# W298/Surtr

Measured on AMD Instinct MI355X. Metric: fragments/sec, higher is better.
Workload: dtype f32

## Files before the change

include/surtr_hip.h:

```cpp
#ifndef SURTR_HIP_H
#define SURTR_HIP_H

#include <stddef.h>
#include <stdint.h>

#ifdef __cplusplus
extern "C" {
#endif

typedef struct surtr_ctx surtr_ctx;

enum {
    SURTR_OK = 0,
    SURTR_E_INVALID = 1,
    SURTR_E_TOPOLOGY = 2,
    SURTR_E_CAPACITY = 3,
    SURTR_E_HIP = 4,
    SURTR_E_STATE = 5,
    SURTR_E_NOGPU = 6
};

enum {
    SURTR_EVT_REFIT = 1,
    SURTR_EVT_RENDER = 2
};

typedef struct surtr_counts {
    uint32_t n_frag;
    uint32_t mesh_verts, mesh_nbrs;
    uint32_t conv_verts, conv_nbrs;
    uint32_t n_idx;
    uint32_t n_pairs;
    uint32_t status;
    uint32_t n_failed;
} surtr_counts;

typedef struct surtr_fragments {
    int32_t* frag_ids;
    uint32_t* mesh_vert_off;
    float* mesh_pos;
    uint32_t* mesh_nbr_off;
    int32_t* mesh_nbr;
    uint32_t* conv_vert_off;
    float* conv_pos;
    uint32_t* conv_nbr_off;
    int32_t* conv_nbr;
    float* vnc;
    uint32_t* idx_off;
    uint32_t* idx;
    uint32_t* frag_status;
} surtr_fragments;

int surtr_create(int device, surtr_ctx** out);
void surtr_destroy(surtr_ctx* ctx);
const char* surtr_strerror(int code);
const char* surtr_last_error(surtr_ctx* ctx);
int surtr_set_stream(surtr_ctx* ctx, void* hip_stream);
int surtr_get_stream(surtr_ctx* ctx, void** hip_stream);
int surtr_set_events_in_flight(surtr_ctx* ctx, uint32_t n);
int surtr_set_scratch(surtr_ctx* ctx, uint32_t max_verts, uint32_t max_nbrs);
int surtr_set_arena(surtr_ctx* ctx, uint64_t verts, uint64_t nbrs, uint64_t idx);

int surtr_set_profiling(surtr_ctx* ctx, int on);
int surtr_kernel_times(surtr_ctx* ctx, float ms[16]);
int surtr_kernel_history(surtr_ctx* ctx, float ms[16], int slot[16], uint32_t* n);
int surtr_queue_stats(surtr_ctx* ctx, uint32_t out[128]);
int surtr_pair_status(surtr_ctx* ctx, uint32_t n_pairs, uint32_t* status);
int surtr_event_pair_costs(surtr_ctx* ctx, uint32_t n_pairs, uint32_t* cost);

int surtr_upload_pieces(surtr_ctx* ctx, uint32_t n_pieces,
                        const uint32_t* mesh_vert_off, const float* mesh_pos,
                        const uint32_t* mesh_nbr_off, const int32_t* mesh_nbr,
                        const uint32_t* conv_vert_off, const float* conv_pos,
                        const uint32_t* conv_nbr_off, const int32_t* conv_nbr);

int surtr_upload_pattern(surtr_ctx* ctx, uint32_t n_cells, const uint32_t* face_off, const float* v012);

int surtr_build_cells(surtr_ctx* ctx, uint32_t n_groups, const uint32_t* group_seed_off, const double* seeds,
                      uint32_t* n_faces, uint32_t* n_face_verts);
int surtr_download_cells(surtr_ctx* ctx, uint32_t* cell_face_off, int32_t* face_gen, uint32_t* face_vert_off, double* verts, float* v012);

int surtr_place_cells(surtr_ctx* ctx, const float scale[3], const float translate[3]);
int surtr_place_cells_impacts(surtr_ctx* ctx, uint32_t n_impacts, const float* scale3, const float* translate3);
int surtr_download_planes(surtr_ctx* ctx, int impacts, uint32_t cap, uint32_t* n, float* planes);

#define SURTR_CELLS_ALL 0xFFFFFFFFu
int surtr_pattern_store(surtr_ctx* ctx, uint32_t* id);
int surtr_pattern_count(surtr_ctx* ctx, uint32_t* n);
int surtr_pattern_info(surtr_ctx* ctx, uint32_t id, uint32_t* n_cells, uint32_t* n_faces);
int surtr_pattern_clear(surtr_ctx* ctx);
int surtr_pattern_select(surtr_ctx* ctx, uint32_t id);
int surtr_place_cells_patterns(surtr_ctx* ctx, uint32_t n_impacts, const uint32_t* pattern_id, const float* scale3, const float* translate3);
int surtr_placed_cells(surtr_ctx* ctx, uint32_t cap, uint32_t* n, uint32_t* cell_base);

int surtr_upload_planes(surtr_ctx* ctx, uint32_t n_cells, const uint32_t* plane_off, const float* planes);

int surtr_fracture_event(surtr_ctx* ctx, uint32_t cell_begin, uint32_t cell_end,
                         const uint8_t* outside, uint32_t flags, surtr_counts* counts);

int surtr_fracture_event_async(surtr_ctx* ctx, uint32_t cell_begin, uint32_t cell_end,
                               const uint8_t* outside, uint32_t flags);
int surtr_event_counts(surtr_ctx* ctx, surtr_counts* counts);

int surtr_fracture_pairs_async(surtr_ctx* ctx, uint32_t n_pairs, const uint32_t* pair_cell, const uint32_t* pair_piece,
                               uint32_t flags);
int surtr_place_cells_groups(surtr_ctx* ctx, uint32_t n_groups, const uint32_t* group_cell_off, const float* scale3,
                             const float* translate3);

int surtr_place_cells_in_pieces(surtr_ctx* ctx, uint32_t n_groups, const uint32_t* group_cell_off);

size_t surtr_event_blob_bytes(const surtr_counts* counts);
int surtr_event_pack_dev(surtr_ctx* ctx, void* dev_blob, size_t capacity_bytes);
int surtr_blob_unpack_host(const void* host_blob, size_t bytes, surtr_counts* counts, surtr_fragments* out);
int surtr_event_download(surtr_ctx* ctx, surtr_fragments* out);

int surtr_clip_polyhedron(surtr_ctx* ctx, uint32_t nv, const float* pos, const uint32_t* nbr_off, const int32_t* nbr,
                          uint32_t n_planes, const float* planes,
                          uint32_t* out_nv, uint32_t* out_nh, float* out_pos, uint32_t* out_nbr_off, int32_t* out_nbr);

int surtr_refit_solid(surtr_ctx* ctx, uint32_t mesh_nv, const float* mesh_pos, const uint32_t* mesh_nbr_off, const int32_t* mesh_nbr,
                      uint32_t conv_nv, const float* conv_pos, const uint32_t* conv_nbr_off, const int32_t* conv_nbr,
                      uint32_t* out_nv, uint32_t* out_nh, float* out_pos, uint32_t* out_nbr_off, int32_t* out_nbr);
int surtr_extract_faces(surtr_ctx* ctx, uint32_t nv, const float* pos, const uint32_t* nbr_off, const int32_t* nbr,
                        uint32_t* n_faces, uint32_t* n_face_idx, uint32_t* face_off, int32_t* face_idx);
int surtr_triangulate(surtr_ctx* ctx, uint32_t nv, const float* pos, const uint32_t* nbr_off, const int32_t* nbr, int is_convex,
                      const float color[3], float* vnc, uint32_t* n_idx, uint32_t* idx);

int surtr_load_fragments(surtr_ctx* ctx, uint32_t n,
                         const uint32_t* mesh_vert_off, const float* mesh_pos, const uint32_t* mesh_nbr_off, const int32_t* mesh_nbr,
                         const uint32_t* conv_vert_off, const float* conv_pos, const uint32_t* conv_nbr_off, const int32_t* conv_nbr,
                         const int32_t* frag_ids);
int surtr_event_triangulate(surtr_ctx* ctx, int is_convex);

int surtr_transform_pieces(surtr_ctx* ctx, uint32_t n_pieces, const float* world);
int surtr_pieces_from_event(surtr_ctx* ctx, const uint8_t* keep, uint32_t* n_pieces);
int surtr_download_piece(surtr_ctx* ctx, uint32_t piece, int set, uint32_t* out_nv, uint32_t* out_nh, float* out_pos,
                         uint32_t* out_nbr_off, int32_t* out_nbr);
enum {
    SURTR_DERIVED_LLEN = 0,
    SURTR_DERIVED_TRI = 1,
    SURTR_DERIVED_RAD = 2,
    SURTR_DERIVED_BOX = 3,
    SURTR_DERIVED_PERM = 4,
    SURTR_DERIVED_POSR_S = 5,
    SURTR_DERIVED_BSPH = 6,
    SURTR_DERIVED_BSPH2 = 7,
    SURTR_DERIVED_BSPH3 = 8,
    SURTR_DERIVED_IPERM = 9,
    SURTR_DERIVED_ROW_S = 10,
    SURTR_DERIVED_DUP = 11,
    SURTR_DERIVED_BO = 12,
    SURTR_DERIVED_BO2 = 13,
    SURTR_DERIVED_BO3 = 14,
    SURTR_DERIVED_BUILD = 15,
    SURTR_DERIVED_COUNT = 16
};
int surtr_pieces_derived(surtr_ctx* ctx, int set, int which, void* out, size_t capacity_bytes, size_t* bytes);
int surtr_upload_stats(surtr_ctx* ctx, float* ms, uint32_t* n_alloc);
int surtr_handover_stats(surtr_ctx* ctx, uint32_t out[8]);
int surtr_regroup_stats(surtr_ctx* ctx, uint32_t out[8]);
int surtr_pair_order(surtr_ctx* ctx, uint32_t cap, uint32_t* n, uint32_t* order);

int surtr_neighbors_from_mesh(uint32_t nv, uint32_t n_tris, const int32_t* tris, uint32_t* nbr_off, int32_t* nbr);

int surtr_neighbors_from_mesh_dev(surtr_ctx* ctx, uint32_t nv, uint32_t n_tris, const int32_t* tris, uint32_t* nbr_off, int32_t* nbr,
                                  float* kernel_ms);

int surtr_voronoi_cells(uint32_t n, const double* seeds, uint32_t* n_faces, uint32_t* n_face_verts,
                        uint32_t* cell_face_off, int32_t* face_gen, uint32_t* face_vert_off, double* verts);

int surtr_hull_normals(uint32_t n, const float* points, uint32_t limit, uint32_t capacity, float* normals, uint32_t* count);

int surtr_kdop_ach_planes(uint32_t n, const float* points, uint32_t k, const float* normals, double max_axis_scale,
                          float plane_gap_inv, float* planes);

int surtr_plane_from_points(const float p0[3], const float p1[3], const float p2[3], float plane[4]);

int surtr_kdop_planes(uint32_t n, const float* points, uint32_t k, const float* normals, float* planes);

int surtr_moments(uint32_t nv, const float* pos, const uint32_t* nbr_off, const int32_t* nbr, double* volume, float centroid[3]);

int surtr_read_obj(const char* path, const float scale[3], const float translate[3], uint32_t cap_verts, uint32_t cap_tris,
                   float* pos, int32_t* tris, uint32_t* n_verts, uint32_t* n_tris);
int surtr_write_obj(const char* path, uint32_t n_frag, const int32_t* frag_ids, const uint32_t* mesh_vert_off, const float* vnc,
                    const uint32_t* idx_off, const uint32_t* idx);

int surtr_convex_out_of_sphere(uint32_t nv, const float* pos, const uint32_t* nbr_off, const int32_t* nbr, uint32_t n_sphere,
                               const float* sphere_points, const float origin[3], float radius, int* out);

int surtr_regroup(uint32_t n_pieces, uint32_t n_outside, const int32_t* piece_cell,
                  const uint32_t* conv_vert_off, const float* conv_pos, const uint32_t* conv_nbr_off, const int32_t* conv_nbr,
                  int partial, uint32_t n_sphere, const float* sphere_points, const float origin[3], float radius,
                  uint32_t* n_compounds, uint32_t* compound_off, int32_t* compound_piece);

int surtr_event_regroup(surtr_ctx* ctx, int partial, uint32_t n_sphere, const float* sphere_points, const float origin[3], float radius,
                        uint32_t* n_pieces, uint32_t* n_compounds, uint32_t* compound_off, int32_t* compound_piece);
int surtr_event_regroup_bodies(surtr_ctx* ctx, int partial, uint32_t n_sphere, const float* sphere_points, const float origin[3], float radius,
                               uint32_t* n_pieces, uint32_t* n_compounds, uint32_t* compound_off, int32_t* compound_piece,
                               uint32_t* n_bodies, uint32_t* body_compound_off);
int surtr_event_regroup_impacts(surtr_ctx* ctx, int partial, uint32_t n_impacts, const uint32_t* sphere_off, const float* sphere_points,
                                const float* origins, const float* radii, uint32_t* n_pieces, uint32_t* n_compounds, uint32_t* compound_off,
                                int32_t* compound_piece, uint32_t* n_bodies, uint32_t* body_compound_off);

int surtr_event_regroup_impacts_partial(surtr_ctx* ctx, const uint8_t* partial, uint32_t n_impacts, const uint32_t* sphere_off, const float* sphere_points,
                                        const float* origins, const float* radii, uint32_t* n_pieces, uint32_t* n_compounds, uint32_t* compound_off,
                                        int32_t* compound_piece, uint32_t* n_bodies, uint32_t* body_compound_off);

int surtr_event_refit(surtr_ctx* ctx);

int surtr_set_refit_point_limit(surtr_ctx* ctx, uint32_t n);
int surtr_get_refit_point_limit(surtr_ctx* ctx, uint32_t* n);
int surtr_hull_normals_device(surtr_ctx* ctx, uint32_t n, const float* points, uint32_t limit, uint32_t capacity, float* normals, uint32_t* count);
int surtr_coord_key(float x, uint32_t* neg, uint64_t* scaled);

typedef struct surtr_mass {
    double volume;
    double mass;
    double com[3];
    double inertia[6];
    uint32_t nv;
    uint32_t status;
} surtr_mass;

int surtr_event_mass_dev(surtr_ctx* ctx, int set, float density, void* dev_out, size_t capacity_bytes);
int surtr_pieces_mass_dev(surtr_ctx* ctx, int set, float density, void* dev_out, size_t capacity_bytes);
int surtr_event_mass(surtr_ctx* ctx, int set, float density, uint32_t* n, surtr_mass* out);
int surtr_pieces_mass(surtr_ctx* ctx, int set, float density, uint32_t* n, surtr_mass* out);
int surtr_combine_mass(uint32_t n_compounds, const uint32_t* compound_off, const int32_t* compound_piece, const surtr_mass* pieces,
                       surtr_mass* out);

typedef struct surtr_ray_hit {
    int32_t piece;
    uint32_t status;
    float t;
    float pos[3];
    float normal[3];
    uint32_t reserved[3];
} surtr_ray_hit;
enum {
    SURTR_RAY_STARTS_INSIDE = 1,
// ... 153 lines not shown
```

surtr_amd/csrc/pieces_dev.hip:

```cpp
#include <chrono>
#include <cstring>

#include "surtr_ctx.h"
#include <hipcub/hipcub.hpp>

namespace {

__device__ __forceinline__ int32_t ring_prev(const int32_t* r, uint32_t len, int32_t who)
{
    uint32_t k = 0;
    while (k < len && r[k] != who) ++k;
    return k == 0 ? r[len - 1] : r[k - 1];
}

__device__ __forceinline__ uint32_t piece_of(const uint32_t* __restrict__ vo, uint32_t n, uint32_t v)
{
    uint32_t lo = 0, hi = n;
    while (hi - lo > 1u) { const uint32_t mid = (lo + hi) >> 1; if (vo[mid] <= v) lo = mid; else hi = mid; }
    return lo;
}

__global__ void k_piece_check(uint32_t V, uint32_t n, const uint32_t* __restrict__ vo, const uint32_t* __restrict__ loff,
                              const int32_t* __restrict__ nbr, uint32_t* __restrict__ llen, uint32_t check, uint32_t* __restrict__ err,
                              uint8_t* __restrict__ dup, uint32_t H)
{
    const uint32_t v = blockIdx.x * blockDim.x + threadIdx.x;
    if (v >= V) return;
    const uint32_t lo = loff[v], hi = loff[v + 1];
    if (hi < lo || hi > H) { atomicMax(err, (uint32_t)SURTR_E_INVALID); llen[v] = 0; return; }
    const uint32_t deg = hi - lo;
    llen[v] = deg;
    const uint32_t p = piece_of(vo, n, v), a = vo[p], m = vo[p + 1] - a;
    for (uint32_t j = lo + 1u; j < hi; ++j)
        for (uint32_t q = lo; q < j; ++q) if (nbr[q] == nbr[j]) { dup[p] = 1; j = hi; break; }
    if (!check) return;
    if (deg < 3u) { atomicMax(err, (uint32_t)SURTR_E_TOPOLOGY); return; }
    const int32_t lv = (int32_t)(v - a);
    for (uint32_t j = lo; j < hi; ++j)
    {
        const int32_t u = nbr[j];
        if (u < 0 || (uint32_t)u >= m || u == lv) { atomicMax(err, (uint32_t)SURTR_E_TOPOLOGY); return; }
        const uint32_t ulo = loff[a + (uint32_t)u], uhi = loff[a + (uint32_t)u + 1];
        if (uhi > H) { atomicMax(err, (uint32_t)SURTR_E_INVALID); return; }
        bool back = false;
        for (uint32_t q = ulo; q < uhi && q >= ulo; ++q) if (nbr[q] == lv) { back = true; break; }
        if (!back) { atomicMax(err, (uint32_t)SURTR_E_TOPOLOGY); return; }
    }
}

__global__ void k_piece_tri_rad(uint32_t V, uint32_t n, const uint32_t* __restrict__ vo, const float* __restrict__ pos,
                                const uint32_t* __restrict__ loff, const int32_t* __restrict__ nbr, uint8_t* __restrict__ tri,
                                float* __restrict__ rad, const uint32_t* __restrict__ gate)
{
    const uint32_t v = blockIdx.x * blockDim.x + threadIdx.x;
    if (v >= V) return;
    if (gate && *gate) return;
    const uint32_t p = piece_of(vo, n, v), a = vo[p], m = vo[p + 1] - a;
    const int32_t lv = (int32_t)(v - a);
    auto ring = [&](int32_t x) { return nbr + loff[a + (uint32_t)x]; };
    auto rlen = [&](int32_t x) { return loff[a + (uint32_t)x + 1] - loff[a + (uint32_t)x]; };
    const uint32_t lo = loff[v], hi = loff[v + 1];
    bool t = true;
    for (uint32_t j = lo; j < hi; ++j)
    {
        const int32_t x = nbr[j];
        const int32_t y = ring_prev(ring(x), rlen(x), lv);
        if (y == lv || ring_prev(ring(y), rlen(y), x) != lv) { t = false; break; }
    }
    tri[v] = t ? 1 : 0;
    const double px = pos[3 * (size_t)v], py = pos[3 * (size_t)v + 1], pz = pos[3 * (size_t)v + 2];
    auto dist = [&](int32_t x) {
        const size_t g = a + (uint32_t)x;
        const double dx = px - (double)pos[3 * g], dy = py - (double)pos[3 * g + 1], dz = pz - (double)pos[3 * g + 2];
        return sqrt(dx * dx + dy * dy + dz * dz);
    };
    double r = 0.0;
    for (uint32_t j = lo; j < hi; ++j)
    {
        const double d = dist(nbr[j]);
        r = d > r ? d : r;
        if (!t)
        {
            int32_t prev = lv, cur = nbr[j]; uint32_t steps = 0;
            while (cur != lv && steps++ < m)
            {
                const double d2 = dist(cur);
                r = d2 > r ? d2 : r;
                const int32_t nx = ring_prev(ring(cur), rlen(cur), prev);
                prev = cur; cur = nx;
            }
        }
    }
    rad[v] = (float)(r * 1.000001) + 1e-30f;
}

__global__ __launch_bounds__(SURTR_WG) void k_piece_box(uint32_t n, const uint32_t* __restrict__ vo, const float* __restrict__ pos, float* __restrict__ box)
{
    __shared__ float part[SURTR_NWAVE][6];
    const uint32_t p = blockIdx.x;
    if (p >= n) return;
    const uint32_t a = vo[p], b = vo[p + 1];
    float lo[3] = {3.0e38f, 3.0e38f, 3.0e38f}, hi[3] = {-3.0e38f, -3.0e38f, -3.0e38f};
    for (uint32_t v = a + threadIdx.x; v < b; v += group_size())
        for (int c = 0; c < 3; ++c) { const float x = pos[3 * (size_t)v + c]; lo[c] = x < lo[c] ? x : lo[c]; hi[c] = x > hi[c] ? x : hi[c]; }
    for (int d = SURTR_LANES / 2; d >= 1; d >>= 1)
        for (int c = 0; c < 3; ++c)
        {
            const float ol = __shfl_down(lo[c], d, SURTR_LANES), oh = __shfl_down(hi[c], d, SURTR_LANES);
            lo[c] = ol < lo[c] ? ol : lo[c]; hi[c] = oh > hi[c] ? oh : hi[c];
        }
    if (lane_id() == 0) for (int c = 0; c < 3; ++c) { part[wave_id()][c] = lo[c]; part[wave_id()][3 + c] = hi[c]; }
    __syncthreads();
    if (threadIdx.x == 0)
    {
        for (uint32_t w = 1; w < group_waves(); ++w)
            for (int c = 0; c < 3; ++c)
            {
                lo[c] = part[w][c] < lo[c] ? part[w][c] : lo[c];
                hi[c] = part[w][3 + c] > hi[c] ? part[w][3 + c] : hi[c];
            }
        for (int c = 0; c < 3; ++c) { box[6 * p + c] = lo[c]; box[6 * p + 3 + c] = hi[c]; }
    }
}

__global__ void k_piece_keys(uint32_t V, uint32_t n, const uint32_t* __restrict__ vo, const float* __restrict__ pos,
                             const float* __restrict__ box, unsigned long long* __restrict__ key, uint32_t* __restrict__ val)
{
    const uint32_t v = blockIdx.x * blockDim.x + threadIdx.x;
    if (v >= V) return;
    const uint32_t p = piece_of(vo, n, v);
// ... 76 lines not shown
        const double dx = s.x - (double)cx, dy = s.y - (double)cy, dz = s.z - (double)cz;
        const double d = sqrt(dx * dx + dy * dy + dz * dz) + (double)s.w;
        R = d > R ? d : R;
    }
    upper[g] = make_float4(cx, cy, cz, (float)(R * 1.000001) + 1e-30f);
}

__global__ void k_piece_iperm(uint32_t V, uint32_t n, const uint32_t* __restrict__ vo, const uint32_t* __restrict__ perm, uint32_t* __restrict__ iperm)
{
    const uint32_t i = blockIdx.x * blockDim.x + threadIdx.x;
    if (i >= V) return;
    const uint32_t p = piece_of(vo, n, i), a = vo[p];
    iperm[a + perm[i]] = i - a;
}
__global__ void k_piece_row_s(uint32_t V, uint32_t n, const uint32_t* __restrict__ vo, const uint32_t* __restrict__ perm,
                              const uint32_t* __restrict__ loff, const uint32_t* __restrict__ llen, const int32_t* __restrict__ nbr,
                              const uint8_t* __restrict__ tri, const uint32_t* __restrict__ iperm, SRow* __restrict__ row_s)
{
    const uint32_t i = blockIdx.x * blockDim.x + threadIdx.x;
    if (i >= V) return;
    const uint32_t p = piece_of(vo, n, i), a = vo[p], m = vo[p + 1] - a;
    const uint32_t g = a + perm[i];
    const uint32_t lo = loff[g], len = llen[g];
    uint32_t h[8];
    h[0] = (len <= 7u ? len : 0x40u) | (tri[g] ? 0u : 0x80u);
    for (uint32_t j = 0; j < 7u; ++j)
    {
        uint32_t e = 0xFFFFu;
        if (len <= 7u && j < len)
        {
            const int32_t u = nbr[lo + j];
            if (u >= 0 && (uint32_t)u < m) { const uint32_t x = iperm[a + (uint32_t)u]; e = x < 0xFFFFu ? x : 0xFFFFu; }
        }
        h[1u + j] = e;
    }
    SRow r;
    for (int q = 0; q < 4; ++q) r.w[q] = h[2 * q] | (h[2 * q + 1] << 16);
    row_s[i] = r;
}

__global__ void k_transform(uint32_t V, uint32_t n, const uint32_t* __restrict__ vo, const float* __restrict__ world, float* __restrict__ pos,
                            uint32_t v0, uint32_t p0)
{
    const uint32_t v = v0 + blockIdx.x * blockDim.x + threadIdx.x;
    if (v >= V) return;
    const float* W = world + 16 * (size_t)(piece_of(vo, n, v) - p0);
    float r[3];
    transform_coord(W, pos[3 * (size_t)v], pos[3 * (size_t)v + 1], pos[3 * (size_t)v + 2], r);
    pos[3 * (size_t)v] = r[0]; pos[3 * (size_t)v + 1] = r[1]; pos[3 * (size_t)v + 2] = r[2];
}

struct FromEvent { const uint32_t* frag; const uint32_t* vo[2]; const uint32_t* ho[2]; };
__global__ __launch_bounds__(SURTR_WG) void k_pieces_from_frags(uint32_t n, FromEvent E, const FragRec* __restrict__ frags, Arena A,
                                                                float* mpos, uint32_t* mloff, int32_t* mnbr, float* cpos, uint32_t* cloff, int32_t* cnbr)
{
    const uint32_t p = blockIdx.x >> 1, set = blockIdx.x & 1u;
    if (p >= n) return;
    const FragRec fr = frags[E.frag[p]];
    const uint32_t sv = set ? fr.cv_off : fr.mv_off, nv = set ? fr.cv_n : fr.mv_n, sh = set ? fr.ch_off : fr.mh_off, nh = set ? fr.ch_n : fr.mh_n;
    const uint32_t dv = E.vo[set][p], dh = E.ho[set][p];
    float* pos = set ? cpos : mpos; uint32_t* loff = set ? cloff : mloff; int32_t* nbr = set ? cnbr : mnbr;
    for (uint32_t i = threadIdx.x; i < 3u * nv; i += group_size()) pos[3 * (size_t)dv + i] = A.pos[3 * (size_t)sv + i];
    for (uint32_t v = threadIdx.x; v < nv; v += group_size()) loff[dv + v] = dh + (A.loff[sv + v] - sh);
    for (uint32_t e = threadIdx.x; e < nh; e += group_size()) nbr[dh + e] = A.nbr[sh + e];
    if (p + 1u == n && threadIdx.x == 0) loff[dv + nv] = dh + nh;
}

static inline uint32_t up_count(uint32_t m) { return (m + SURTR_SPH_FAN - 1u) / SURTR_SPH_FAN; }

}

namespace pieces {

int reserve_set(surtr_ctx* ctx, PieceSet& S, uint32_t n, uint32_t V, uint32_t H, uint32_t NB)
{
    if (grow_pieces(ctx, S.pos, 3 * (size_t)V + 3) || grow_pieces(ctx, S.loff, (size_t)V + 1) || grow_pieces(ctx, S.llen, V) ||
        grow_pieces(ctx, S.nbr, (size_t)H + 1) || grow_pieces(ctx, S.vo, n + 1) || grow_pieces(ctx, S.tri, V) || grow_pieces(ctx, S.rad, V) ||
        grow_pieces(ctx, S.perm, V) || grow_pieces(ctx, S.posr_s, (size_t)V + 1) || grow_pieces(ctx, S.bsph, NB + 1) ||
        grow_pieces(ctx, S.bo, n + 1) || grow_pieces(ctx, S.box, 6 * (size_t)n) || grow_pieces(ctx, S.key, V) || grow_pieces(ctx, S.key2, V) ||
        grow_pieces(ctx, S.val, V) || grow_pieces(ctx, S.dup, n + 1) || grow_pieces(ctx, S.iperm, V) || grow_pieces(ctx, S.row_s, (size_t)V + 1) ||
        grow_pieces(ctx, S.bsph2, (size_t)NB / SURTR_SPH_FAN + n + 1) || grow_pieces(ctx, S.bo2, n + 1) ||
        grow_pieces(ctx, S.bsph3, (size_t)NB / (SURTR_SPH_FAN * SURTR_SPH_FAN) + n + 1) || grow_pieces(ctx, S.bo3, n + 1))
        return SURTR_E_HIP;
    return SURTR_OK;
}

int derive_set(surtr_ctx* ctx, PieceSet& S, uint32_t n, uint32_t V, const std::vector<uint32_t>& bo_h, bool check, uint32_t H)
{
    hipStream_t st = ctx->stream;
    const uint32_t NB = bo_h[n];
    HIPCHK(hipMemcpyAsync(S.bo, bo_h.data(), (size_t)(n + 1) * 4, hipMemcpyHostToDevice, st));
    const dim3 blk(256), gridV((V + 255) / 256);
    HIPCHK(hipMemsetAsync(S.dup, 0, (size_t)n + 1, st));
    hipLaunchKernelGGL(k_piece_check, gridV, blk, 0, st, V, n, S.vo, S.loff, S.nbr, S.llen, check ? 1u : 0u, ctx->d_upload_err, S.dup, check ? H : 0xFFFFFFFFu);
    hipLaunchKernelGGL(k_piece_tri_rad, gridV, blk, 0, st, V, n, S.vo, S.pos, S.loff, S.nbr, S.tri, S.rad,
                       check ? (const uint32_t*)ctx->d_upload_err.p : (const uint32_t*)nullptr);
    hipLaunchKernelGGL(k_piece_box, dim3(n), dim3(SURTR_WG), 0, st, n, S.vo, S.pos, S.box);
    hipLaunchKernelGGL(k_piece_keys, gridV, blk, 0, st, V, n, S.vo, S.pos, S.box, S.key, S.val);
    int end_bit = 32;
    while (end_bit < 64 && (n >> (end_bit - 32)) != 0u) ++end_bit;
    size_t tmp_bytes = 0;
    if (hipcub::DeviceRadixSort::SortPairs(nullptr, tmp_bytes, S.key.p, S.key2.p, S.val.p, S.perm.p, (int)V, 0, end_bit, st) != hipSuccess) return SURTR_E_HIP;
    int rc = grow_pieces(ctx, ctx->sort_tmp, tmp_bytes + 16);
    if (rc) return rc;
    if (hipcub::DeviceRadixSort::SortPairs(ctx->sort_tmp.p, tmp_bytes, S.key.p, S.key2.p, S.val.p, S.perm.p, (int)V, 0, end_bit, st) != hipSuccess) return SURTR_E_HIP;
    hipLaunchKernelGGL(k_piece_sorted, gridV, blk, 0, st, V, n, S.vo, S.pos, S.rad, S.perm, S.posr_s);
    if (NB) hipLaunchKernelGGL(k_piece_spheres, dim3((NB + 255) / 256), blk, 0, st, NB, n, S.vo, S.bo, S.posr_s, S.bsph);
    std::vector<uint32_t> bo2(n + 1, 0u), bo3(n + 1, 0u);
    for (uint32_t p = 0; p < n; ++p) { bo2[p + 1] = bo2[p] + up_count(bo_h[p + 1] - bo_h[p]); bo3[p + 1] = bo3[p] + up_count(bo2[p + 1] - bo2[p]); }
    HIPCHK(hipMemcpyAsync(S.bo2, bo2.data(), (size_t)(n + 1) * 4, hipMemcpyHostToDevice, st));
    HIPCHK(hipMemcpyAsync(S.bo3, bo3.data(), (size_t)(n + 1) * 4, hipMemcpyHostToDevice, st));
    if (bo2[n]) hipLaunchKernelGGL(k_piece_spheres_up, dim3((bo2[n] + 255) / 256), blk, 0, st, bo2[n], n, S.bo, S.bo2, S.bsph, S.bsph2);
    if (bo3[n]) hipLaunchKernelGGL(k_piece_spheres_up, dim3((bo3[n] + 255) / 256), blk, 0, st, bo3[n], n, S.bo2, S.bo3, S.bsph2, S.bsph3);
    hipLaunchKernelGGL(k_piece_iperm, gridV, blk, 0, st, V, n, S.vo, S.perm, S.iperm);
    hipLaunchKernelGGL(k_piece_row_s, gridV, blk, 0, st, V, n, S.vo, S.perm, S.loff, S.llen, S.nbr, S.tri, S.iperm, S.row_s);
    HIPCHK(hipGetLastError());
    return SURTR_OK;
}

int host_offsets(uint32_t n, const uint32_t* vo, const uint32_t* off, std::vector<uint32_t>& ho)
{
    if (vo[0] != 0) return SURTR_E_INVALID;
    for (uint32_t p = 0; p < n; ++p)
    {
        const uint32_t a = vo[p], b = vo[p + 1];
        if (b < a || b - a < 4 || b - a >= (1u << 24)) return SURTR_E_INVALID;
        if (off[b] < off[a]) return SURTR_E_INVALID;
    }
    ho.resize(n + 1);
    for (uint32_t p = 0; p <= n; ++p) ho[p] = off[vo[p]];
    return SURTR_OK;
}

int vet_solids(surtr_ctx* ctx, uint32_t n, uint32_t V, uint32_t H, const uint32_t* vo, const uint32_t* loff, const int32_t* nbr, uint32_t* llen, uint8_t* dup)
{
    hipStream_t st = ctx->stream;
    HIPCHK(hipMemsetAsync(dup, 0, (size_t)n + 1, st));
    hipLaunchKernelGGL(k_piece_check, dim3((V + 255) / 256), dim3(256), 0, st, V, n, vo, loff, nbr, llen, 1u, ctx->d_upload_err.p, dup, H);
    HIPCHK(hipGetLastError());
    return SURTR_OK;
}

std::vector<uint32_t> sphere_offsets(uint32_t n, const uint32_t* vo)
{
    std::vector<uint32_t> bo(n + 1, 0u);
    for (uint32_t p = 0; p < n; ++p) bo[p + 1] = bo[p] + (vo[p + 1] - vo[p] + SURTR_SB - 1u) / SURTR_SB;
    return bo;
}

void set_piece_stats(surtr_ctx* ctx, uint32_t n, const uint32_t* mvo, const uint32_t* mho, const uint32_t* cvo, const uint32_t* cho)
{
    uint32_t vmax = 0, hmax = 0, cvmax = 0, chmax = 0, small = 0, vmin = 0xFFFFFFFFu;
    for (uint32_t i = 0; i < n; ++i)
    {
        vmax = std::max(vmax, mvo[i + 1] - mvo[i]); vmin = std::min(vmin, mvo[i + 1] - mvo[i]); hmax = std::max(hmax, mho[i + 1] - mho[i]);
        cvmax = std::max(cvmax, cvo[i + 1] - cvo[i]); chmax = std::max(chmax, cho[i + 1] - cho[i]);
        if (surtr_fits_half((mvo[i + 1] - mvo[i]) / 4u, (mho[i + 1] - mho[i]) / 4u)) ++small;
    }
    ctx->vmin = n ? vmin : 0u;
    ctx->n_pieces = n; ctx->vmax = std::max(vmax, cvmax); ctx->hmax = std::max(hmax, chmax); ctx->cvmax = cvmax; ctx->chmax = chmax;
    ctx->tot_mv = mvo[n]; ctx->tot_mh = mho[n]; ctx->pair_order_count = 0;
    ctx->half_on = 4ull * small >= 3ull * n;
    if (const char* e = getenv("SURTR_HALF")) ctx->half_on = atoi(e) != 0;
    ctx->have_event = false; ctx->frags_of_pieces = false;
    ctx->scene_off.assign({0u, n}); ctx->scene_event_compound.clear();
    scene_reset_poses(ctx);
    ctx->h_vo[0].assign(mvo, mvo + n + 1); ctx->h_ho[0].assign(mho, mho + n + 1);
    ctx->h_vo[1].assign(cvo, cvo + n + 1); ctx->h_ho[1].assign(cho, cho + n + 1);
}

int finish_upload(surtr_ctx* ctx, uint32_t n, bool check)
{
    const int rc = grow_pieces(ctx, ctx->d_outside, n);
    if (rc) return rc;
    uint32_t err = 0;
    HIPCHK(hipMemcpyAsync(&err, ctx->d_upload_err, 4, hipMemcpyDeviceToHost, ctx->stream));
    HIPCHK(hipStreamSynchronize(ctx->stream));
    if (check && err) { ctx->n_pieces = 0; return (int)err; }
    return SURTR_OK;
// ... 144 lines not shown
    if (g >= n) return;
    for (int c = 0; c < 3; ++c)
    {
        const float lo = box[6 * g + c], hi = box[6 * g + 3 + c];
        scale3[3 * g + c] = hi - lo;
        shift3[3 * g + c] = (float)(((double)hi + (double)lo) / 2.0);
    }
}

int surtr_place_cells_in_pieces(surtr_ctx* ctx, uint32_t n_groups, const uint32_t* group_cell_off)
{
    if (!ctx || !n_groups || !group_cell_off) return SURTR_E_INVALID;
    if (!ctx->n_pieces || !ctx->d_v012) return SURTR_E_STATE;
    if (n_groups != ctx->n_pieces) return SURTR_E_INVALID;
    (void)hipSetDevice(ctx->device);
    int rc = grow_pieces(ctx, ctx->d_group_xf, (size_t)6 * n_groups);
    if (rc) return rc;
    float* sc = ctx->d_group_xf; float* sh = sc + 3 * (size_t)n_groups;
    hipLaunchKernelGGL(k_group_boxes, dim3((n_groups + 255) / 256), dim3(256), 0, ctx->stream, n_groups, ctx->mset.box, sc, sh);
    HIPCHK(hipGetLastError());
    return surtr_place_cells_groups_dev(ctx, n_groups, group_cell_off, sc, sh);
}

int surtr_download_piece(surtr_ctx* ctx, uint32_t piece, int set, uint32_t* out_nv, uint32_t* out_nh, float* out_pos, uint32_t* out_off, int32_t* out_nbr)
{
    if (!ctx || set < 0 || set > 1) return SURTR_E_INVALID;
    if (!ctx->n_pieces) return SURTR_E_STATE;
    if (piece >= ctx->n_pieces) return SURTR_E_INVALID;
    (void)hipSetDevice(ctx->device);
    const PieceSet& S = set ? ctx->cset : ctx->mset;
    HIPCHK(hipStreamSynchronize(ctx->stream));
    uint32_t vo[2], ho[2];
    HIPCHK(hipMemcpy(vo, S.vo + piece, 8, hipMemcpyDeviceToHost));
    HIPCHK(hipMemcpy(&ho[0], S.loff + vo[0], 4, hipMemcpyDeviceToHost));
    HIPCHK(hipMemcpy(&ho[1], S.loff + vo[1], 4, hipMemcpyDeviceToHost));
    const uint32_t nv = vo[1] - vo[0], nh = ho[1] - ho[0];
    if (out_nv) *out_nv = nv;
    if (out_nh) *out_nh = nh;
    if (out_pos) HIPCHK(hipMemcpy(out_pos, S.pos + 3 * (size_t)vo[0], (size_t)nv * 12, hipMemcpyDeviceToHost));
    if (out_off)
    {
        HIPCHK(hipMemcpy(out_off, S.loff + vo[0], ((size_t)nv + 1) * 4, hipMemcpyDeviceToHost));
        for (uint32_t v = 0; v <= nv; ++v) out_off[v] -= ho[0];
    }
    if (out_nbr && nh) HIPCHK(hipMemcpy(out_nbr, S.nbr + ho[0], (size_t)nh * 4, hipMemcpyDeviceToHost));
    return SURTR_OK;
}

int surtr_upload_stats(surtr_ctx* ctx, float* ms, uint32_t* n_alloc)
{
    if (!ctx) return SURTR_E_INVALID;
    if (ms) *ms = ctx->upload_ms;
    if (n_alloc) *n_alloc = ctx->upload_allocs;
    return SURTR_OK;
}

int surtr_handover_stats(surtr_ctx* ctx, uint32_t out[8])
{
    if (!ctx || !out) return SURTR_E_INVALID;
    (void)hipSetDevice(ctx->device);
    HIPCHK(hipStreamSynchronize(ctx->stream));
    if (ctx->stream2) HIPCHK(hipStreamSynchronize(ctx->stream2));
    if (ctx->stream3) HIPCHK(hipStreamSynchronize(ctx->stream3));
    uint32_t c[CUR_HO_WORDS] = {};
    if (ctx->arena.cursors) HIPCHK(hipMemcpy(c, ctx->arena.cursors + CUR_HO_PUSHED, sizeof(c), hipMemcpyDeviceToHost));
    for (uint32_t k = 0; k < CUR_HO_WORDS; ++k) out[k] = c[k];
    out[6] = ctx->max_wg;
    out[7] = (uint32_t)ctx->d_hlist.cap;
    return SURTR_OK;
}

int surtr_pair_order(surtr_ctx* ctx, uint32_t cap, uint32_t* n, uint32_t* order)
{
    if (!ctx || !n) return SURTR_E_INVALID;
    (void)hipSetDevice(ctx->device);
    *n = ctx->d_pair_order ? ctx->pair_order_count : 0u;
    if (!order || *n == 0u) return SURTR_OK;
    if (cap < *n) return SURTR_E_CAPACITY;
    HIPCHK(hipStreamSynchronize(ctx->stream));
    HIPCHK(hipMemcpy(order, ctx->d_pair_order, (size_t)*n * 4, hipMemcpyDeviceToHost));
    return SURTR_OK;
}

int surtr_pieces_derived(surtr_ctx* ctx, int set, int which, void* out, size_t capacity_bytes, size_t* bytes)
{
    if (!ctx || set < 0 || set > 1 || !bytes || which < 0 || which >= SURTR_DERIVED_COUNT) return SURTR_E_INVALID;
    const uint32_t build[2] = {SURTR_SB, SURTR_SPH_FAN};
    const void* src = nullptr; size_t b = 0;
    if (which == SURTR_DERIVED_BUILD) b = sizeof(build);
    else
    {
        if (!ctx->n_pieces) return SURTR_E_STATE;
        const PieceSet& S = set ? ctx->cset : ctx->mset;
        const uint32_t n = ctx->n_pieces; const size_t V = ctx->h_vo[set][n];
        const std::vector<uint32_t> bo = sphere_offsets(n, ctx->h_vo[set].data());
        size_t nb2 = 0, nb3 = 0;
        for (uint32_t p = 0; p < n; ++p) { const uint32_t a = up_count(bo[p + 1] - bo[p]); nb2 += a; nb3 += up_count(a); }
        switch (which)
        {
        case SURTR_DERIVED_LLEN:   src = S.llen.p;   b = V * 4; break;
        case SURTR_DERIVED_TRI:    src = S.tri.p;    b = V; break;
        case SURTR_DERIVED_RAD:    src = S.rad.p;    b = V * 4; break;
        case SURTR_DERIVED_BOX:    src = S.box.p;    b = (size_t)n * 24; break;
        case SURTR_DERIVED_PERM:   src = S.perm.p;   b = V * 4; break;
        case SURTR_DERIVED_POSR_S: src = S.posr_s.p; b = V * 16; break;
        case SURTR_DERIVED_BSPH:   src = S.bsph.p;   b = (size_t)bo[n] * 16; break;
        case SURTR_DERIVED_BSPH2:  src = S.bsph2.p;  b = nb2 * 16; break;
        case SURTR_DERIVED_BSPH3:  src = S.bsph3.p;  b = nb3 * 16; break;
        case SURTR_DERIVED_IPERM:  src = S.iperm.p;  b = V * 4; break;
        case SURTR_DERIVED_ROW_S:  src = S.row_s.p;  b = V * 16; break;
        case SURTR_DERIVED_DUP:    src = S.dup.p;    b = n; break;
        case SURTR_DERIVED_BO:     src = S.bo.p;     b = ((size_t)n + 1) * 4; break;
        case SURTR_DERIVED_BO2:    src = S.bo2.p;    b = ((size_t)n + 1) * 4; break;
        default:                   src = S.bo3.p;    b = ((size_t)n + 1) * 4; break;
        }
    }
    *bytes = b;
    if (!out) return SURTR_OK;
    if (capacity_bytes < b) return SURTR_E_CAPACITY;
    if (!src) { memcpy(out, build, b); return SURTR_OK; }
    (void)hipSetDevice(ctx->device);
    HIPCHK(hipStreamSynchronize(ctx->stream));
    if (b) HIPCHK(hipMemcpy(out, src, b, hipMemcpyDeviceToHost));
    return SURTR_OK;
}

}
```

surtr_amd/csrc/small_clip.h:

```cpp
#pragma once
#include "clip_core.h"

#define SC_V 192u
#define SC_H 640u
#define SC_FALLBACK 101

namespace surtr {

template <uint32_t CAPV, uint32_t CAPH, class WORD = uint32_t>
struct ScSolidT
{
    typedef WORD Word;
    static constexpr uint32_t kVwSh = sizeof(WORD) == 4 ? 16u : 12u, kReSh = sizeof(WORD) == 4 ? 16u : 8u;
    static_assert(CAPV <= (1u << kReSh) && CAPH <= (1u << kVwSh), "a vertex id / a ring offset fits its field");
    float pos[3 * CAPV];
    WORD vw[CAPV];
    WORD re[CAPH];
};
typedef ScSolidT<SC_V, SC_H> ScSolid;

template <uint32_t CAPV, uint32_t CAPH, class WORD = uint32_t>
struct ScLdsT
{
    static_assert(CAPV % 4u == 0 && CAPV <= 0x7FFFu && CAPH <= 0xFFFFu, "16-bit indices, 4-byte arrays");
    static constexpr uint32_t kV = CAPV, kH = CAPH;
    typedef ScSolidT<CAPV, CAPH, WORD> Solid;
    Solid buf[2];
    int8_t c[CAPV];
    uint16_t km[CAPV];
    uint16_t mp[CAPV];
    uint16_t noff[CAPV];
    uint16_t succ[CAPV], pred[CAPV];
    uint32_t nv[2], flag;
#ifdef SURTR_STAMP
    unsigned long long tph[8];
#endif
};
typedef ScLdsT<SC_V, SC_H> ScLds;

template <class SH, class LDS>
__device__ inline int small_clip(const SolidIn in, const uint32_t F, const SH& sh, LDS& L, uint32_t* which, uint32_t* stop = nullptr)
{
    typedef typename LDS::Solid ScSolid;
    constexpr uint32_t CAPV = LDS::kV, CAPH = LDS::kH;
    constexpr uint32_t VS = ScSolid::kVwSh, VM = (1u << VS) - 1u, RS = ScSolid::kReSh, RM = (1u << RS) - 1u;
    const uint32_t lane = lane_id();
    const uint32_t V = in.nv;
#ifdef SURTR_STAMP
    unsigned long long sc_t0 = __builtin_readcyclecounter();
    if (lane == 0) for (int q = 0; q < 8; ++q) L.tph[q] = 0;
#define SC_STAMP(i) do { if (lane == 0) { const unsigned long long t1 = __builtin_readcyclecounter(); L.tph[i] += t1 - sc_t0; sc_t0 = t1; } } while (0)
#else
#define SC_STAMP(i) do { } while (0)
#endif
    if (stop != nullptr) *stop = 0xFFFFFFFFu;
    if (V == 0 || V > CAPV) return SC_FALLBACK;
    const uint32_t hbase = in.loff[0], H = in.loff[V - 1u] + in.llen[V - 1u] - hbase;
    if (H > CAPH) return SC_FALLBACK;
    bool odd = false;
    for (uint32_t v = lane; v < V; v += SURTR_LANES)
    {
        ScSolid& S = L.buf[0];
        S.pos[3 * v] = in.pos[3 * v]; S.pos[3 * v + 1] = in.pos[3 * v + 1]; S.pos[3 * v + 2] = in.pos[3 * v + 2];
        const uint32_t lo = in.loff[v] - hbase, deg = in.llen[v];
        if (deg > 15u || deg < 3u) odd = true;
        const uint32_t dl = deg > 15u ? 15u : deg;
        S.vw[v] = lo | (dl << VS);
        const int32_t* r = in.nbr + in.loff[v];
        for (uint32_t j = 0; j < dl && lo + j < CAPH; ++j)
        {
            if ((uint32_t)r[j] >= V) odd = true;
            S.re[lo + j] = (uint32_t)r[j] & RM;
            for (uint32_t jj = 0; jj < j; ++jj) if (r[jj] == r[j]) odd = true;
        }
    }
    if (__ballot(odd) != 0ull) return SC_FALLBACK;
    __syncthreads();
    for (uint32_t v = lane; v < V; v += SURTR_LANES)
    {
        ScSolid& S = L.buf[0];
        const uint32_t w = S.vw[v], lo = w & VM, deg = w >> VS;
        for (uint32_t j = 0; j < deg; ++j)
        {
            const uint32_t e = S.re[lo + j] & RM;
            const uint32_t we = S.vw[e], elo = we & VM, edeg = we >> VS;
            uint32_t q = 0;
            while (q < edeg && (S.re[elo + q] & RM) != v) ++q;
            if (q >= edeg) odd = true;
            S.re[lo + j] = e | (q << RS);
        }
    }
    if (__ballot(odd) != 0ull) return SC_FALLBACK;
    __syncthreads();
    SC_STAMP(0);
#define SC_GIVE_UP do { if (stop != nullptr) { *stop = k; *which = cur; if (lane == 0) L.nv[cur] = nv; __syncthreads(); } return SC_FALLBACK; } while (0)
    uint32_t cur = 0, nv = V;
    for (uint32_t k = 0; k < F && nv != 0u; ++k)
    {
        const float4 pl = sh.planes[k];
        ScSolid& S = L.buf[cur]; ScSolid& N = L.buf[cur ^ 1u];
        bool zero = false, cut = false, keep = false;
        for (uint32_t v = lane; v < nv; v += SURTR_LANES)
        {
            const int c = side_of(plane_dist(pl, S.pos[3 * v], S.pos[3 * v + 1], S.pos[3 * v + 2]));
            L.c[v] = (int8_t)c;
            zero = zero || c == 0; cut = cut || c < 0; keep = keep || c > 0;
        }
        const bool anyCut = __ballot(cut) != 0ull;
        if (__ballot(keep) == 0ull) { if (!anyCut) SC_GIVE_UP; nv = 0; break; }
        if (!anyCut) continue;
        if (__ballot(zero) != 0ull) SC_GIVE_UP;
        __syncthreads();
        SC_STAMP(1);
        uint32_t carryM = 0, carryK = 0, carryH = 0;
        for (uint32_t v0 = 0; v0 < nv; v0 += SURTR_LANES)
        {
            const uint32_t v = v0 + lane;
            uint32_t mask = 0, isKept = 0, deg = 0;
            if (v < nv)
            {
                const uint32_t w = S.vw[v], lo = w & VM;
                deg = w >> VS;
                if (L.c[v] > 0) isKept = 1u;
                else
                    for (uint32_t j = 0; j < deg; ++j) if (L.c[S.re[lo + j] & RM] > 0) mask |= 1u << j;
            }
            const uint32_t cnt = (uint32_t)__builtin_popcount(mask);
            const uint2 inc = wave_incl_scan2(make_uint2(cnt | (isKept << 16), isKept ? deg : 0u));
            if (v < nv)
            {
                L.km[v] = (uint16_t)mask;
                L.mp[v] = isKept ? (uint16_t)(carryK + (inc.x >> 16) - 1u) : (uint16_t)(0x8000u | (carryM + (inc.x & 0xFFFFu) - cnt));
                L.noff[v] = (uint16_t)(carryH + inc.y - (isKept ? deg : 0u));
            }
            const uint32_t tx = lane_bcast(inc.x, SURTR_LANES - 1u), ty = lane_bcast(inc.y, SURTR_LANES - 1u);
            carryM += tx & 0xFFFFu; carryK += tx >> 16; carryH += ty;
        }
        const uint32_t M = carryM, nKeep = carryK, HK = carryH;
        if (nKeep + M > CAPV || HK + 3u * M > CAPH) SC_GIVE_UP;
        if (nKeep + M < 4u) { nv = 0; break; }
        for (uint32_t t = lane; t < M; t += SURTR_LANES) L.pred[t] = 0xFFFFu;
        __syncthreads();
        SC_STAMP(2);
        bool bad = false;
        for (uint32_t v = lane; v < nv; v += SURTR_LANES)
        {
            uint32_t mask = L.c[v] < 0 ? L.km[v] : 0u;
            if (!mask) continue;
            uint32_t t = L.mp[v] & 0x7FFFu;
            const uint32_t wv = S.vw[v];
            for (; mask; mask &= mask - 1u, ++t)
            {
                uint32_t cv = v, w = wv, slot = (uint32_t)__builtin_ctz(mask), steps = 0, end = 0xFFFFu;
                while (steps++ <= nv)
                {
                    const uint32_t len = w >> VS;
                    const uint32_t p = slot == 0u ? len - 1u : slot - 1u;
                    const uint32_t rw = S.re[(w & VM) + p];
                    const uint32_t e = rw & RM;
                    if (L.c[e] > 0) { end = (L.mp[cv] & 0x7FFFu) + (uint32_t)__builtin_popcount(L.km[cv] & ((1u << p) - 1u)); break; }
                    cv = e; slot = rw >> RS; w = S.vw[e];
                }
                if (end == 0xFFFFu || end == t) { bad = true; continue; }
                L.succ[t] = (uint16_t)end;
                L.pred[end] = (uint16_t)t;
            }
        }
        if (__ballot(bad) != 0ull) SC_GIVE_UP;
        __syncthreads();
        SC_STAMP(3);
        for (uint32_t t = lane; t < M; t += SURTR_LANES) if (L.pred[t] == 0xFFFFu || L.pred[L.succ[t]] != t || L.pred[t] == L.succ[t]) bad = true;
        if (__ballot(bad) != 0ull) SC_GIVE_UP;
        SC_STAMP(4);
        for (uint32_t v = lane; v < nv; v += SURTR_LANES)
        {
            const uint32_t w = S.vw[v], lo0 = w & VM, deg = w >> VS;
            if (L.c[v] > 0)
// ... 95 lines not shown
```

surtr_amd/csrc/surtr_ctx.h:

```cpp
#pragma once
#include <algorithm>
#include <chrono>
#include <cstdint>
#include <cstdlib>
#include <string>
#include <vector>

#include "../../include/surtr_hip.h"
#include "clip_core.h"

using namespace surtr;

struct PairRec
{
    uint32_t cv_off, cv_n, ch_off, ch_n;
    uint32_t mv_off, mv_n, mh_off, mh_n;
    uint32_t ni, isl_off;
    uint32_t status;
    uint32_t img_fmt, img_off, img_n, img_h, img_pc;
    uint32_t cv_bad;
};

enum { IMG_NONE = 0,
       IMG_NARROW = 1,
// ... 30 lines not shown
    uint32_t mv_off, mv_n, mh_off, mh_n;
    uint32_t cv_off, cv_n, ch_off, ch_n;
    uint32_t idx_off, idx_n;
    uint32_t o_mv, o_mh, o_cv, o_ch, o_idx;
};

struct Arena
{
    float* pos; uint32_t* loff; uint32_t* llen; int32_t* nbr; uint32_t* idx;
    uint2* isl;
    uint32_t capV, capH, capI, capIsl;
    uint32_t* cursors;
};

enum : uint32_t
{
    CUR_V = 0,
    CUR_H = 1,
    CUR_I = 2,
    CUR_ISL = 3,
    CUR_Q_CLIP = 4,
    CUR_STATUS = 5,
    CUR_Q_REFIT = 6,
    CUR_Q_FACES = 7,
    CUR_Q_CONVEX = 8,
    CUR_Q_PREP = 9,
    CUR_IMG = 10,
    CUR_Q_BIG = 11,
    CUR_Q_HALF = 12,
    CUR_Q_RETRY = 13,
    CUR_FLAGGED_FRAGS = 14,
    CUR_FLAGGED_PAIRS = 15,
    CUR_CLS_CLIP = 16,
    CUR_CLS_FRAG = 32,
    CUR_CLS_PREP = 48,
    CUR_CLS_HALF = 64,
    CUR_RETRY_N = CUR_CLS_HALF,
    CUR_CVX_RESUMED = 78,
    CUR_REFIT_RESUMED = 79,
    CUR_CVX_TOOK = 80,
    CUR_REFIT_TOOK = 82,
    CUR_BIG_QUOTA = 84,
    CUR_FACES2_N = 85,
    CUR_Q_FACES2 = 86,
    CUR_CVX_GAVE_UP = 87,
    CUR_REC_TOOK = 88,
    CUR_REC_HANDED = 89,
    CUR_LIT_TOO_LARGE = 90,
    CUR_REC_IMAGES = 91,
    CUR_SORTED_SEL = 92,
    CUR_REC_SPENT = 93,
    CUR_CATCH_CLIPPED = 94,
    CUR_UNREFITTED = 95,
    CUR_WC_WHY = 96,
    CUR_Q_CONVEX2 = 125,
    CUR_STATS_WORDS = 128,
    CUR_HO_PUSHED = 146,
    CUR_HO_STARTED = 147,
    CUR_HO_SIGNED_OFF = 148,
    CUR_HO_POLL_SLOT = 149,
    CUR_Q_CATCH = 150,
    CUR_Q_SWEEP = 151,
    CUR_HO_WORDS = 6,
    CUR_COUNT = 256
};
static_assert(CUR_V == 0 && CUR_H == 1 && CUR_I == 2 && CUR_ISL == 3 && CUR_STATUS == 5 && CUR_CLS_CLIP == 16 && CUR_CLS_FRAG == 32 &&
              CUR_CLS_PREP == 48 && CUR_CLS_HALF == 64 && CUR_REC_TOOK == 88 && CUR_REC_HANDED == 89 && CUR_LIT_TOO_LARGE == 90 &&
              CUR_UNREFITTED == 95 && CUR_WC_WHY == 96, "include/surtr_hip.h publishes these slots of surtr_queue_stats by number");
static_assert(CUR_STATS_WORDS <= CUR_COUNT && CUR_Q_SWEEP + 1 == CUR_HO_PUSHED + CUR_HO_WORDS && CUR_HO_PUSHED + CUR_HO_WORDS <= CUR_COUNT &&
              CUR_Q_FACES2 == CUR_FACES2_N + 1, "slot map");

struct alignas(16) SRow { uint32_t w[4]; };

struct Pieces
{
    const float* mpos; const uint32_t* mloff; const uint32_t* mllen; const int32_t* mnbr; const uint32_t* mvo; const uint8_t* mtri; const float* mrad;
    const uint32_t* mperm; const float4* mposr_s; const float4* mbsph; const uint32_t* mbo;
    const float* cpos; const uint32_t* cloff; const uint32_t* cllen; const int32_t* cnbr; const uint32_t* cvo; const uint8_t* ctri; const float* crad;
    const uint32_t* cperm; const float4* cposr_s; const float4* cbsph; const uint32_t* cbo;
    uint32_t n;
    const uint8_t* mdup; const uint8_t* cdup;
    const SRow* mrow_s; const uint32_t* miperm;
    const float4* mbsph2; const uint32_t* mbo2; const float4* mbsph3; const uint32_t* mbo3;
};

struct ScratchPool
{
    char* base; size_t per_wg;
    uint32_t CV, CH, VMAX;
};

struct Scratch
{
    float* pos;
    uint32_t* g_loff; uint32_t* g_llen; int8_t* g_comp; uint32_t* g_ring;
    uint32_t* g_succ; uint32_t* g_pred; uint32_t* g_pcnt;
    uint32_t* aux0; uint32_t* aux1; uint32_t* aux2; uint32_t* aux3;
    int8_t* g_gcomp;
    uint2* blk;
    unsigned long long* gmask; uint2* gblk;
    float* t_pos; uint32_t* t_loff; uint32_t* t_llen; int8_t* t_comp; uint32_t* t_ring;
    uint32_t CV, CH;
};

__device__ static Scratch carve(const ScratchPool& P, uint32_t wg)
{
    Scratch S;
    char* p = P.base + (size_t)wg * P.per_wg;
    auto take = [&](size_t bytes) { char* r = p; p += (bytes + 255) & ~(size_t)255; return r; };
    S.pos = (float*)take((size_t)P.CV * 12);
    S.g_loff = (uint32_t*)take((size_t)P.CV * 4);
    S.g_llen = (uint32_t*)take((size_t)P.CV * 4);
    S.g_comp = (int8_t*)take((size_t)P.CV);
    S.g_ring = (uint32_t*)take((size_t)P.CH * 4);
    S.g_succ = (uint32_t*)take((size_t)P.CV * 4);
    S.g_pred = (uint32_t*)take((size_t)P.CV * 4);
    S.g_pcnt = (uint32_t*)take((size_t)P.CV * 4);
    const size_t AV = P.CV > P.VMAX ? P.CV : P.VMAX;
    S.aux0 = (uint32_t*)take(AV * 4);
    S.aux1 = (uint32_t*)take((size_t)P.CV * 4);
    S.aux2 = (uint32_t*)take(AV * 4);
    S.aux3 = (uint32_t*)take((size_t)P.CV * 4);
    S.g_gcomp = (int8_t*)take((size_t)P.CV);
    S.blk = (uint2*)take((size_t)(P.CV / SURTR_LANES + 4) * 8);
    S.gmask = (unsigned long long*)take((size_t)(P.VMAX / SURTR_LANES + 2) * 8);
    S.gblk = (uint2*)take((size_t)(P.VMAX / SURTR_LANES + 2) * 8);
    S.t_pos = (float*)take((size_t)P.CV * 12); S.t_loff = (uint32_t*)take((size_t)P.CV * 4); S.t_llen = (uint32_t*)take((size_t)P.CV * 4);
    S.t_comp = (int8_t*)take((size_t)P.CV); S.t_ring = (uint32_t*)take((size_t)P.CH * 4);
    S.CV = P.CV; S.CH = P.CH;
    return S;
}

static size_t scratch_bytes_per_wg(uint32_t CV, uint32_t CH, uint32_t VMAX)
{
    auto r = [](size_t b) { return (b + 255) & ~(size_t)255; };
    return 2 * r((size_t)CV * 12) + 9 * r((size_t)CV * 4) + 2 * r((size_t)std::max(CV, VMAX) * 4) + 3 * r((size_t)CV) + 2 * r((size_t)CH * 4) + r((size_t)(CV / SURTR_LANES + 4) * 8) +
           2 * r((size_t)(VMAX / SURTR_LANES + 2) * 8);
}

struct FaceScratch
{
    int32_t* base; size_t per_wg; uint32_t HF;
};

struct surtr_ctx;

template <class T>
struct DevBuf
{
    T* p = nullptr;
    size_t cap = 0;
    DevBuf() = default;
    DevBuf(DevBuf&& o) noexcept : p(o.p), cap(o.cap) { o.p = nullptr; o.cap = 0; }
    DevBuf& operator=(DevBuf&& o) noexcept { if (this != &o) { reset(); p = o.p; cap = o.cap; o.p = nullptr; o.cap = 0; } return *this; }
    ~DevBuf() { reset(); }
    void reset() { if (p) (void)hipFree(p); p = nullptr; cap = 0; }
    operator T*() const { return p; }
    int grow(surtr_ctx* ctx, size_t need, size_t alloc = 0);
};

struct PieceSet
{
    DevBuf<float> pos; DevBuf<uint32_t> loff, llen; DevBuf<int32_t> nbr; DevBuf<uint32_t> vo; DevBuf<uint8_t> tri; DevBuf<float> rad;
    DevBuf<uint32_t> perm; DevBuf<float4> posr_s, bsph; DevBuf<uint32_t> bo;
    DevBuf<float> box; DevBuf<unsigned long long> key, key2; DevBuf<uint32_t> val;
    DevBuf<uint8_t> dup;
    DevBuf<uint32_t> iperm; DevBuf<SRow> row_s;
    DevBuf<float4> bsph2; DevBuf<uint32_t> bo2; DevBuf<float4> bsph3; DevBuf<uint32_t> bo3;
};

struct CellBuffers
{
    DevBuf<double> seeds; DevBuf<uint32_t> goff; DevBuf<char> slots; DevBuf<uint32_t> cfo, cvo;
    DevBuf<int32_t> gen; DevBuf<uint32_t> fvo; DevBuf<double> verts; DevBuf<uint32_t> heads;
    uint32_t n = 0, nf = 0, nfv = 0;
};

#define SURTR_LVS (SURTR_LV / 2u)
#define SURTR_LHS ((SURTR_LH * 11u / 24u) & ~7u)
#ifndef SURTR_HALF_ROOM
#define SURTR_HALF_ROOM 2u
#endif
__host__ __device__ static inline bool fits_half(uint32_t n, uint32_t h, uint32_t capVs) { return SURTR_HALF_ROOM * n <= capVs && SURTR_HALF_ROOM * h <= SURTR_LHS; }
static inline bool surtr_fits_half(uint32_t n, uint32_t h) { return fits_half(n, h, SURTR_LVS); }

struct surtr_ctx
{
    int device = 0;
    bool frags_of_pieces = false;
    uint32_t hw_wg = 512, hw_wg_faces = 1024, hw_wg_prep = 1792, hw_wg_big = 48, budget_vmax = 0xFFFFFFFFu, budget_hmax = 0xFFFFFFFFu;
    uint32_t max_wg = 512, max_wg_faces = 1024, max_wg_small = 2048, max_wg_lean = 3072, max_wg_prep = 1792, max_wg_half = 1024;
    DevBuf<uint32_t> d_hlist;
    uint32_t vmin = 0;
    ScratchPool pool_half{}; uint32_t n_wg_half = 0; DevBuf<char> pool_half_buf;
    bool half_on = false;
    PrepPool prep{nullptr, 0, 0}; uint32_t n_wg_prep = 0; DevBuf<char> prep_buf;
    ImgArena img{nullptr, 0}; DevBuf<char> img_buf;
    DevBuf<uint32_t> d_order;
    DevBuf<uint32_t> d_forder;
    bool wave_big = false;
    uint32_t n_wg_big = 48;
    hipStream_t stream2 = nullptr;
    hipStream_t stream3 = nullptr;
    hipEvent_t ev_prep = nullptr, ev_big = nullptr, ev_half = nullptr, ev_cvx = nullptr;
    uint32_t events_in_flight = 1;
    hipStream_t stream = nullptr;
    std::string err;
    uint32_t n_pieces = 0, vmax = 0, hmax = 0, cvmax = 0, chmax = 0;
    CellBuffers cells;
    PieceSet mset, cset;
    DevBuf<uint32_t> d_upload_err;
    DevBuf<float> d_group_xf;
    DevBuf<float> d_world;
    DevBuf<char> sort_tmp;
    DevBuf<uint32_t> d_from;
    DevBuf<uint32_t> d_qstatus; uint32_t qstatus_n = 0;
    float upload_ms = 0.f; uint32_t upload_allocs = 0;
    std::vector<uint32_t> scene_off;
    std::vector<uint32_t> h_vo[2], h_ho[2];
    std::vector<uint32_t> scene_event_compound;
    std::vector<uint32_t> scene_event_impacts;
    DevBuf<uint32_t> d_outside_list;
    std::vector<uint32_t> h_outside_stage;
    std::vector<float> scene_pose;
    bool scene_dev_stale = true;
    std::vector<double> h_pose_stage; std::vector<uint32_t> h_comp_stage;
    DevBuf<double> d_pose;
    DevBuf<uint32_t> d_piece_comp;
    struct { DevBuf<float> pos; DevBuf<uint32_t> loff; DevBuf<int32_t> nbr; DevBuf<uint32_t> vo; } spare[2];
    DevBuf<int32_t> d_commit_src; DevBuf<uint32_t> d_commit_tab;
    DevBuf<float> d_posef; bool scene_posef_stale = true; std::vector<float> h_posef_stage;
    DevBuf<surtr_bounds> d_bounds_piece;
    DevBuf<char> d_cull;
    struct { DevBuf<float> pos; DevBuf<uint32_t> loff, llen, vo; DevBuf<int32_t> nbr; DevBuf<uint8_t> dup; } stage[2];
    std::vector<uint32_t> h_frag_stage; DevBuf<uint32_t> d_frag_tab;
    float commit_ms[2] = {0.f, 0.f};
    uint32_t regroup_rounds = 0;
    uint64_t tot_mv = 0, tot_mh = 0;
    uint32_t n_cells = 0, n_faces = 0;
    DevBuf<uint32_t> d_cvx_giveup;
    DevBuf<uint32_t> d_pair_order; uint32_t pair_order_begin = 0, pair_order_count = 0;
    bool pair_order_is_list = false;
    DevBuf<float> d_v012; DevBuf<float4> d_planes; DevBuf<uint32_t> d_plane_off;
    std::vector<uint32_t> h_plane_off;
    bool planes_ready = false;
    uint32_t n_impacts_placed = 0;
    DevBuf<float4> d_planes_imp; DevBuf<uint32_t> d_plane_off_imp; DevBuf<float> d_imp_xf;
    std::vector<uint32_t> h_plane_off_imp; std::vector<float> h_imp_xf;
    bool imp_library = false; std::vector<uint32_t> imp_cell_base; uint32_t imp_faces = 0;
    DevBuf<uint32_t> d_imp_tab; std::vector<uint32_t> h_imp_tab;
    struct LibPattern { uint32_t n_cells, n_faces, face_base, off_base; };
// ... 218 lines not shown
```

surtr_amd/csrc/surtr_hip.hip:

```cpp
#include <algorithm>
#include <cmath>
#include <cstdio>
#include <cstdlib>
#include <cstring>
#include <string>
#include <type_traits>
#include <vector>

#include "surtr_ctx.h"
#include "small_clip.h"
#ifndef SC_RESUME
#define SC_RESUME 1
#endif
#include "literal_clip.h"
#include "wave_clip.h"
#include "prep_sorted.h"

template <uint32_t LV, uint32_t LH>
struct alignas(16) LdsTopoT
{
    static_assert(LV % 16 == 0 && LH % 8 == 0, "clip_image copies 16-byte words into these arrays");
    static constexpr uint32_t kLV = LV, kLH = LH;
    alignas(16) uint16_t loff[LV];
    alignas(16) uint8_t llen[LV];
// ... 197 lines not shown
    const uint32_t f = blockIdx.x * blockDim.x + threadIdx.x;
    if (f >= nfaces) return;
    const uint32_t g = face_group[f];
    const float sx = scale3[3 * g], sy = scale3[3 * g + 1], sz = scale3[3 * g + 2];
    const float tx = shift3[3 * g], ty = shift3[3 * g + 1], tz = shift3[3 * g + 2];
    planes[f] = placed_plane(v012 + 9 * f, sx, sy, sz, tx, ty, tz);
}

__global__ void k_place_cells_impacts(uint32_t nfaces, uint32_t n_imp, const float* __restrict__ v012, const float* __restrict__ scale3,
                                      const float* __restrict__ shift3, float4* __restrict__ planes)
{
    const uint32_t f = blockIdx.x * blockDim.x + threadIdx.x;
    if (f >= nfaces) return;
    float v[9];
    for (int i = 0; i < 9; ++i) v[i] = v012[9 * (size_t)f + i];
    for (uint32_t g = 0; g < n_imp; ++g)
    {
        const float sx = scale3[3 * g], sy = scale3[3 * g + 1], sz = scale3[3 * g + 2];
        const float tx = shift3[3 * g], ty = shift3[3 * g + 1], tz = shift3[3 * g + 2];
        planes[(size_t)g * nfaces + f] = placed_plane(v, sx, sy, sz, tx, ty, tz);
    }
}

__global__ void k_place_cells_patterns(uint32_t ntotal, uint32_t n_imp, const uint32_t* __restrict__ face_prefix, const uint32_t* __restrict__ lib_face_base,
                                       const float* __restrict__ lib_v012, const float* __restrict__ scale3, const float* __restrict__ shift3,
                                       float4* __restrict__ planes)
{
    const uint32_t g = blockIdx.x * blockDim.x + threadIdx.x;
    if (g >= ntotal) return;
    uint32_t lo = 0, hi = n_imp;
    while (hi - lo > 1u)
    {
        const uint32_t mid = lo + (hi - lo) / 2u;
        if (face_prefix[mid] <= g) lo = mid; else hi = mid;
    }
    const uint32_t f = g - face_prefix[lo];
    const float* src = lib_v012 + 9 * ((size_t)lib_face_base[lo] + f);
    float v[9];
    for (int i = 0; i < 9; ++i) v[i] = src[i];
    const float sx = scale3[3 * lo], sy = scale3[3 * lo + 1], sz = scale3[3 * lo + 2];
    const float tx = shift3[3 * lo], ty = shift3[3 * lo + 1], tz = shift3[3 * lo + 2];
    planes[g] = placed_plane(v, sx, sy, sz, tx, ty, tz);
}

__device__ __forceinline__ void pair_failed(const Arena& A, int err)
{
    if (err == SURTR_E_TOPOLOGY) atomicAdd(&A.cursors[CUR_FLAGGED_PAIRS], 1u); else atomicMax(&A.cursors[CUR_STATUS], (uint32_t)err);
}

__device__ __forceinline__ uint32_t pair_of_ticket(const Arena& A, const uint32_t* __restrict__ table, uint32_t n_pairs, uint32_t& t, uint32_t class_base,
                                                   int cls_hi, int cls_lo)
{
    uint32_t p = 0xFFFFFFFFu;
    for (int cls = cls_hi; cls >= cls_lo; --cls)
    {
        const uint32_t cnt = A.cursors[class_base + cls];
        if (t < cnt) { p = table[(size_t)cls * n_pairs + t]; break; }
        t -= cnt;
    }
    return p;
}
__device__ __forceinline__ uint32_t take_pair(const Arena& A, const uint32_t* __restrict__ table, uint32_t n_pairs, uint32_t ticket_slot, uint32_t class_base,
                                              int cls_hi, int cls_lo)
{
    uint32_t t = atomicAdd(&A.cursors[ticket_slot], 1u);
    return pair_of_ticket(A, table, n_pairs, t, class_base, cls_hi, cls_lo);
}
struct PairAt { uint32_t cell, piece; };
__device__ __forceinline__ PairAt pair_where(uint32_t p, const uint2* __restrict__ pair_list, uint32_t cell_begin, uint32_t n_pieces)
{
    return PairAt{pair_list ? pair_list[p].x : cell_begin + p / n_pieces, pair_list ? pair_list[p].y : p % n_pieces};
}
__device__ __forceinline__ SolidIn mesh_solid_in(const Pieces& P, uint32_t piece)
{
    const uint32_t m0 = P.mvo[piece];
    return SolidIn{P.mpos + 3 * (size_t)m0, P.mloff + m0, P.mllen + m0, P.mnbr, P.mvo[piece + 1] - m0, P.mtri + m0, P.mrad + m0,
                   P.mperm + m0, P.mposr_s + m0, P.mbsph + P.mbo[piece]};
}
__device__ __forceinline__ SolidIn convex_solid_in(const Pieces& P, uint32_t piece)
{
    const uint32_t c0 = P.cvo[piece];
    return SolidIn{P.cpos + 3 * (size_t)c0, P.cloff + c0, P.cllen + c0, P.cnbr, P.cvo[piece + 1] - c0, P.ctri + c0, P.crad + c0,
                   P.cperm + c0, P.cposr_s + c0, P.cbsph + P.cbo[piece]};
}
__device__ __forceinline__ int finish_pair(const Arena& A, PairRec* __restrict__ pairs, uint32_t p, PairRec& rec, int err)
{
    if (err == 0 && rec.cv_bad != 0 && rec.ni != 0) err = SURTR_E_TOPOLOGY;
    if (err != 0) { rec.status = (uint32_t)err; rec.ni = 0; if (threadIdx.x == 0) pair_failed(A, err); }
    if (threadIdx.x == 0) pairs[p] = rec;
    return err;
}

__device__ __attribute__((always_inline)) static inline bool arena_take(const Arena& A, Shared& sh, uint32_t nv, uint32_t nh, uint32_t nisl,
                                  uint32_t& voff, uint32_t& hoff, uint32_t& ioff)
{
    __syncthreads();
    if (threadIdx.x == 0)
    {
        sh.misc[0] = atomicAdd(&A.cursors[CUR_V], nv);
        sh.misc[1] = atomicAdd(&A.cursors[CUR_H], nh);
        sh.misc[2] = nisl ? atomicAdd(&A.cursors[CUR_ISL], nisl) : 0u;
    }
    __syncthreads();
    voff = sh.misc[0]; hoff = sh.misc[1]; ioff = sh.misc[2];
    const bool ok = (uint64_t)voff + nv <= A.capV && (uint64_t)hoff + nh <= A.capH && (uint64_t)ioff + nisl <= A.capIsl;
    __syncthreads();
    return ok;
}

template <class TT>
__device__ __attribute__((always_inline)) static inline int park_topo(Topo<TT>& T, Shared& sh, const Arena& A, uint32_t& voff, uint32_t& n, uint32_t& hoff, uint32_t& nh)
{
    const uint2 tot = index_live(T, sh);
    uint32_t ioff;
    if (!arena_take(A, sh, tot.x, tot.y, 0, voff, hoff, ioff)) return SURTR_E_CAPACITY;
    write_solid(T, A.pos, A.loff, A.llen, A.nbr, voff, hoff);
    n = tot.x; nh = tot.y;
    __syncthreads();
    return 0;
}

template <class TT>
__device__ __attribute__((always_inline)) static inline int park_mesh_islands(Topo<TT>& T, Shared& sh, const Arena& A, PairRec& rec)
{
    typedef typename TT::idx_t I;
    const uint32_t tid = threadIdx.x, nS = T.nS;
    STAMP_DECL;
    if (sizeof(I) == 2)
    {
        const uint32_t nA = select_count(T.fc, SURTR_NEVER, nS, sh);
        uint32_t wtop = T.capH;
        auto carve = [&](uint32_t n) -> uint16_t* {
            if (wtop < T.hUsed + n + 8u) return nullptr;
            wtop -= n; return (uint16_t*)(void*)(T.ring + wtop);
        };
        uint16_t* alist = carve(nA); uint16_t* lab = carve(nS); uint16_t* pidx = carve(nS); uint16_t* roff = carve(nA + 1u);
        if (alist && lab && pidx && roff && T.hUsed < 0xFFFFu)
        {
            select_write(T.fc, SURTR_NEVER, nS, sh, WArr<uint16_t>{alist, nullptr});
            for (uint32_t i = tid; i < nA; i += group_size()) { const uint32_t v = alist[i]; lab[v] = (uint16_t)v; pidx[v] = (uint16_t)i; }
            __syncthreads();
            while (true)
            {
                if (tid == 0) sh.changed = 0;
                __syncthreads();
                bool ch = false;
                for (uint32_t i = tid; i < nA; i += group_size())
                {
                    const uint32_t v = alist[i];
                    uint32_t m = lab[v];
                    const I* r = T.ring + T.loff[v];
                    const uint32_t len = T.llen[v];
                    for (uint32_t q = 0; q < len; ++q) { const uint32_t o = lab[(uint32_t)r[q]]; m = o < m ? o : m; }
                    const uint32_t mm = lab[m];
                    m = mm < m ? mm : m;
                    if (m < lab[v]) { lab[v] = (uint16_t)m; ch = true; }
                }
                if (ch) sh.changed = 1;
                __syncthreads();
                const bool more = sh.changed != 0;
                __syncthreads();
                if (!more) break;
            }
            if (tid == 0) sh.changed = 0;
            __syncthreads();
            {
// ... 149 lines not shown
}

__device__ __forceinline__ static bool solid_is_sliver_inl(const SolidIn& in)
{
    bool odd = false;
    for (uint32_t v = threadIdx.x; v < in.nv; v += group_size())
    {
        const int32_t* r = in.nbr + in.loff[v];
        const uint32_t deg = in.llen[v];
        for (uint32_t j = 0; j < deg; ++j)
        {
            const int32_t u = r[j];
            for (uint32_t q = 0; q < j; ++q) if (r[q] == u) odd = true;
            if (u < 0 || (uint32_t)u >= in.nv) { odd = true; continue; }
            const int32_t* ru = in.nbr + in.loff[u];
            const uint32_t du = in.llen[u];
            bool back = false;
            for (uint32_t q = 0; q < du; ++q) if (ru[q] == (int32_t)v) back = true;
            if (!back) odd = true;
        }
    }
    return __syncthreads_or(odd ? 1 : 0) != 0;
}
__device__ static bool solid_is_sliver(const SolidIn in) { return solid_is_sliver_inl(in); }

struct LitRun { int err; uint32_t n, nh; LitSolid LS; const uint32_t* off; bool stale; };
__device__ __attribute__((noinline)) static LitRun literal_run(SolidIn in, uint32_t F, ScratchPool pool, uint32_t wg, Shared* shp, bool ids_set = false,
                                                                uint32_t* too_big = nullptr)
{
    Shared& sh = *shp;
    Scratch S = carve(pool, wg);
    const uint32_t capV = S.CV < S.CH / LIT_STRIDE ? S.CV : S.CH / LIT_STRIDE;
    LitRun r{SURTR_E_TOPOLOGY, 0u, 0u, LitSolid{S.pos, S.g_loff, (int32_t*)S.g_ring, S.g_llen, (int32_t*)S.t_ring, S.g_comp, (int32_t*)S.aux0, capV}, S.aux1, false};
    __syncthreads();
    if (threadIdx.x == 0)
    {
        uint32_t n = 0; bool stale = false;
        int rc = literal_clip(in, F, sh.planes, r.LS, &n, &stale, ids_set);
        if (rc == SURTR_E_CAPACITY) { rc = SURTR_E_TOPOLOGY; if (too_big != nullptr) atomicAdd(too_big, 1u); }
        uint32_t h = 0;
        if (rc == 0) for (uint32_t v = 0; v < n; ++v) { S.aux1[v] = h; h += r.LS.len[v]; }
        sh.misc[2] = (uint32_t)rc; sh.misc[3] = n; sh.misc[4] = h; sh.misc[5] = stale ? 1u : 0u;
    }
    __syncthreads();
    r.err = (int)sh.misc[2]; r.n = sh.misc[3]; r.nh = sh.misc[4]; r.stale = sh.misc[5] != 0u;
    __syncthreads();
    return r;
}
__device__ static void literal_write(const LitRun& r, float* pos, uint32_t* loff, uint32_t* llen, int32_t* nbr, uint32_t voff, uint32_t hoff)
{
    for (uint32_t v = threadIdx.x; v < r.n; v += group_size())
    {
        const size_t id = (size_t)voff + v;
        pos[3 * id] = r.LS.pos[3 * v]; pos[3 * id + 1] = r.LS.pos[3 * v + 1]; pos[3 * id + 2] = r.LS.pos[3 * v + 2];
        const uint32_t lo = hoff + r.off[v], len = r.LS.len[v];
        loff[id] = lo; llen[id] = len;
        for (uint32_t q = 0; q < len; ++q) nbr[lo + q] = r.LS.ring[v * LIT_STRIDE + q];
    }
    __syncthreads();
}
__device__ __attribute__((noinline)) static ParkOut solid_literal(SolidIn in, uint32_t F, ScratchPool pool, uint32_t wg, Arena A, Shared* shp, bool ids_set = false)
{
    const LitRun r = literal_run(in, F, pool, wg, shp, ids_set, &A.cursors[CUR_LIT_TOO_LARGE]);
    ParkOut o{r.err, 0u, 0u, 0u, 0u, r.stale};
    if (r.err != 0 || r.n == 0u) return o;
    uint32_t ioff;
    if (!arena_take(A, *shp, r.n, r.nh, 0, o.voff, o.hoff, ioff)) { o.err = SURTR_E_CAPACITY; return o; }
    literal_write(r, A.pos, A.loff, A.llen, A.nbr, o.voff, o.hoff);
    o.n = r.n; o.nh = r.nh;
    return o;
}

struct ChainCaller
{
    uint32_t slot_took, slot_resumed;
    bool count_literal_first;
    float4* keep;
    const float4* restore_from;
};
struct LiteralArg { SolidIn in; bool ids_set; };
struct ChainStamp { unsigned long long t_small, t_park; int path; };
template <class Literal>
__device__ __forceinline__ ParkOut convex_chain(const SolidIn cin, const uint32_t F, bool literal_first, const ChainCaller who, Literal&& literal,
                                                Shared& sh, OneWaveLds& U, Scratch& S, const ScratchPool& pool, const Arena& A, ChainStamp& st)
{
    const uint32_t tid = threadIdx.x;
    ParkOut o{SURTR_E_TOPOLOGY, 0u, 0u, 0u, 0u, false};
    uint32_t which = 0, stop = 0xFFFFFFFFu;
#ifdef SURTR_NO_SMALL_CLIP
    literal_first = false;
    o.err = SC_FALLBACK;
#else
    if (!literal_first) o.err = small_clip(cin, F, sh, U.f, &which, &stop);
#endif
    if (tid == 0 && (!literal_first || who.count_literal_first)) atomicAdd(&A.cursors[who.slot_took + (o.err == 0 ? 0u : 1u)], 1u);
#ifdef SURTR_STAMP
    st.t_small = st.t_park = __builtin_readcyclecounter();
#endif
    if (!literal_first)
    {
        if (o.err == 0)
        {
            const uint32_t nv = U.f.nv[which];
            if (nv != 0u) o.err = sc_park(U.f.buf[which], nv, sh, A.cursors, A.pos, A.loff, A.llen, A.nbr, A.capV, A.capH, o.voff, o.n, o.hoff, o.nh);
        }
        __syncthreads();
#ifdef SURTR_STAMP
        st.t_park = __builtin_readcyclecounter();
#endif
        if (o.err == SC_FALLBACK)
        {
            SolidIn cx = cin; uint32_t Fx = F;
            const bool resumed = SC_RESUME && stop != 0xFFFFFFFFu && stop > 0u && stop < F;
            if (resumed)
            {
                const uint32_t nvs = U.f.nv[which];
                cx = sc_stage(U.f.buf[which], nvs, S.pos, S.g_loff, S.g_llen, S.g_ring);
                Fx = F - stop;
                for (uint32_t k = tid; k < F; k += group_size())
                {
                    const float4 pk = sh.planes[k];
                    if (who.keep != nullptr) who.keep[k] = pk;
                    sh.pmar[k] = pk;
                }
                __syncthreads();
                for (uint32_t k = tid; k < Fx; k += group_size()) sh.planes[k] = sh.pmar[k + stop];
                __syncthreads();
                if (tid == 0) atomicAdd(&A.cursors[who.slot_resumed], 1u);
            }
            o.err = clip_any<false>(cx, Fx, S, sh, U.g.L, [&](auto& T) -> int {
                if (T.nLive == 0) return 0;
                return park_topo(T, sh, A, o.voff, o.n, o.hoff, o.nh);
            }, &U.g.W);
            __syncthreads();
            if (resumed)
            {
                for (uint32_t k = tid; k < F; k += group_size()) sh.planes[k] = who.restore_from[k];
                __syncthreads();
            }
        }
#ifdef SURTR_STAMP
        if (o.err == SURTR_OVERFLOW) st.path |= 1;
        if (o.err == SURTR_E_TOPOLOGY) st.path |= 2;
#endif
        if (o.err == SURTR_OVERFLOW)
        {
            o = solid_global(cin, F, pool, blockIdx.x, A, &sh);
            __syncthreads();
        }
    }
    if (o.err == SURTR_E_TOPOLOGY)
    {
#ifdef SURTR_STAMP
        st.path |= 4;
#endif
        const LiteralArg la = literal();
        const ParkOut l = solid_literal(la.in, F, pool, blockIdx.x, A, &sh, la.ids_set);
        if (l.err == 0) o = l;
        else if (l.err != SURTR_E_TOPOLOGY) o.err = l.err;
        __syncthreads();
    }
    return o;
}

#ifndef SURTR_LITERAL_MESH_V
#define SURTR_LITERAL_MESH_V 2048u
#define SURTR_LITERAL_START_V 64u
#endif
#ifndef SURTR_SMALL_WAVES
#define SURTR_SMALL_WAVES 2
#endif
__device__ __forceinline__ static void convex_publish(PairRec* __restrict__ pairs, uint32_t p, const PairRec& rec, uint32_t front_par)
{
    if (threadIdx.x != 0) return;
    if (!front_par) pairs[p] = rec;
    else
// ... 15 lines not shown
    {
        const float4 pk = planes[k];
        const float n1 = fabsf(pk.x) + fabsf(pk.y) + fabsf(pk.z);
        const float n2 = sqrtf(pk.x * pk.x + pk.y * pk.y + pk.z * pk.z) * 1.0001f;
        pmar[k] = make_float4(n2 * 1.00101f, 1.0e-5f * fabsf(pk.w), 1.0e-5f * n1, 0.f);
    }
    __syncthreads();
    uint32_t und = 0;
    for (uint32_t sb = tid * 8u; sb < nsb; sb += group_size() * 8u)
    {
        const float4 sp = bs[sb];
        const float mag = fabsf(sp.x) + fabsf(sp.y) + fabsf(sp.z) + sp.w;
        bool decided = false;
        for (uint32_t k = 0; k < F; ++k)
        {
            const float4 mk = pmar[k];
            const float sk = plane_dist(planes[k], sp.x, sp.y, sp.z);
            const float margin = sp.w * mk.x + mk.y + mk.z * mag;
            if (sk > margin) { decided = true; break; }
            if (!(sk < -margin)) break;
        }
        if (!decided) ++und;
    }
    const uint2 tot = wave_incl_scan2(make_uint2(und, 0u));
    if (tid == group_size() - 1u)
    {
        uint32_t l2 = 0; while ((tot.x >> (l2 + 1u)) != 0u) ++l2;
        uint32_t cls = 2u * l2 + (l2 ? ((tot.x >> (l2 - 1u)) & 1u) : 0u);
        cls = cls > 4u ? cls - 4u : 0u; if (cls > 15u) cls = 15u;
        porder[(size_t)cls * n_pairs + atomicAdd(&A.cursors[CUR_CLS_PREP + cls], 1u)] = p;
    }
}

__global__ __launch_bounds__(SURTR_LANES) __attribute__((amdgpu_waves_per_eu(SURTR_SMALL_WAVES, 8))) void k_clip_convex(Pieces P, const float4* __restrict__ planes,
                                                    const uint32_t* __restrict__ plane_off, uint32_t cell_begin,
                                                    uint32_t n_pairs, const uint8_t* __restrict__ outside,
                                                    ScratchPool pool, Arena A, PairRec* __restrict__ pairs,
                                                    const uint2* __restrict__ pair_list, uint32_t* __restrict__ porder,
                                                    const uint32_t* __restrict__ pair_order, uint32_t front_par,
                                                    const uint32_t* __restrict__ giveup)
{
    __shared__ Shared sh;
    __shared__ OneWaveLds U;
    LdsTopoSmall& L = U.g.L; LdsWorkSmall& W = U.g.W;
    Scratch S = carve(pool, blockIdx.x);
    const uint32_t tid = threadIdx.x;
    while (true)
    {
        __syncthreads();
        if (tid == 0)
        {
            if (giveup == nullptr) sh.misc[7] = atomicAdd(&A.cursors[CUR_Q_CONVEX], 1u);
            else
            {
                const uint32_t t = atomicAdd(&A.cursors[CUR_Q_CONVEX2], 1u);
                sh.misc[7] = t < A.cursors[CUR_CVX_GAVE_UP] ? giveup[t] : 0xFFFFFFFFu;
            }
        }
        __syncthreads();
        uint32_t p = sh.misc[7];
        if (p >= n_pairs) break;
        if (giveup == nullptr && pair_order != nullptr) p = pair_order[p];
        const PairAt at = pair_where(p, pair_list, cell_begin, P.n);
        const uint32_t cell = at.cell, piece = at.piece;
        PairRec rec;
        memset(&rec, 0, sizeof(rec));
#ifdef SURTR_STAMP_SMALL
        if (tid == 0) for (int q = 0; q < 16; ++q) sh.ph[q] = 0;
#endif
        bool skip = outside != nullptr && outside[piece] != 0;
        const uint32_t f0 = plane_off[cell], F = plane_off[cell + 1] - f0;
        if (F > SURTR_MAXF) { rec.status = SURTR_E_INVALID; skip = true; }
        int err = 0;
        ChainStamp cst{};
#ifdef SURTR_STAMP
        const unsigned long long cx0 = __builtin_readcyclecounter();
        cst.t_small = cst.t_park = cx0;
#endif
        if (!skip)
        {
            for (uint32_t k = tid; k < F; k += group_size()) sh.planes[k] = planes[f0 + k];
            __syncthreads();
            const ChainCaller who{CUR_CVX_TOOK, CUR_CVX_RESUMED, true, nullptr, planes + f0};
            const ParkOut o = convex_chain(convex_solid_in(P, piece), F, P.cdup[piece] != 0, who, [&] { return LiteralArg{convex_solid_in(P, piece), false}; }, sh, U, S, pool, A, cst);
            err = o.err; rec.cv_off = o.voff; rec.cv_n = o.n; rec.ch_off = o.hoff; rec.ch_n = o.nh;
        }
        if (err == SURTR_E_TOPOLOGY) { rec.cv_bad = 1; rec.cv_off = 0; rec.cv_n = 1; rec.ch_off = 0; rec.ch_n = 0; err = 0; }
        if (err != 0) { rec.status = (uint32_t)err; rec.cv_n = 0; if (tid == 0) atomicMax(&A.cursors[CUR_STATUS], (uint32_t)err); }
        convex_publish(pairs, p, rec, front_par);
        if (rec.cv_n != 0 && porder != nullptr) convex_enqueue_prep(P, piece, p, F, sh.planes, sh.pmar, A, porder, n_pairs);
#ifdef SURTR_STAMP_SMALL
        if (tid == 0) for (int q = 0; q < 16; ++q) if (sh.ph[q]) atomicAdd(&g_stamp[q], sh.ph[q]);
#endif
#ifdef SURTR_STAMP
        if (tid == 0)
        {
            const unsigned long long cx1 = cst.t_small, cx2 = cst.t_park, cx3 = __builtin_readcyclecounter();
            const unsigned long long d = cx3 - cx0;
            atomicAdd(&g_stamp2[32], d); atomicAdd(&g_stamp2[33], 1ull);
            const unsigned long long old = atomicMax(&g_stamp2[34], d);
            if (d > old)
            {
                g_stamp2[35] = cx1 - cx0; g_stamp2[36] = cx2 - cx1; g_stamp2[37] = cx3 - cx2; g_stamp2[38] = F;
                for (int q = 0; q < 7; ++q) g_stamp2[40 + q] = U.f.tph[q];
            }
        }
#endif
    }
}

#ifndef SURTR_LEAN_WAVES
#define SURTR_LEAN_WAVES 2
#endif
#ifndef SURTR_LEAN_V
#if SURTR_LEAN_WAVES <= 2
#define SURTR_LEAN_V SC_V
#define SURTR_LEAN_H SC_H
#define SURTR_LEAN_WORD uint32_t
#elif SURTR_LEAN_WAVES == 3
#define SURTR_LEAN_V SC_V
#define SURTR_LEAN_H SC_H
#define SURTR_LEAN_WORD uint16_t
#else
#define SURTR_LEAN_V 156u
#define SURTR_LEAN_H 480u
#define SURTR_LEAN_WORD uint16_t
#endif
#endif
struct LeanShared { float4 planes[SURTR_MAXF + 1]; uint32_t misc[8]; };
typedef ScLdsT<SURTR_LEAN_V, SURTR_LEAN_H, SURTR_LEAN_WORD> LeanSolidLds;
union alignas(16) LeanLds { LeanSolidLds f; float4 pmar[SURTR_MAXF + 1]; };
#if SURTR_LANES != 1
static_assert((sizeof(LeanShared) + sizeof(LeanLds)) * 4u * SURTR_LEAN_WAVES <= 160u * 1024u, "LDS admits fewer workgroups per CU than the register budget");
#endif
__global__ __launch_bounds__(SURTR_LANES) __attribute__((amdgpu_waves_per_eu(SURTR_LEAN_WAVES, 8))) void k_clip_convex_lean(Pieces P, const float4* __restrict__ planes,
                                                    const uint32_t* __restrict__ plane_off, uint32_t cell_begin,
                                                    uint32_t n_pairs, const uint8_t* __restrict__ outside,
                                                    Arena A, PairRec* __restrict__ pairs,
                                                    const uint2* __restrict__ pair_list, uint32_t* __restrict__ porder,
                                                    const uint32_t* __restrict__ pair_order, uint32_t front_par,
                                                    uint32_t* __restrict__ giveup)
{
    __shared__ LeanShared sh;
    __shared__ LeanLds U;
    const uint32_t tid = threadIdx.x;
    while (true)
    {
        __syncthreads();
        if (tid == 0) sh.misc[7] = atomicAdd(&A.cursors[CUR_Q_CONVEX], 1u);
        __syncthreads();
        uint32_t p = sh.misc[7];
        if (p >= n_pairs) break;
        if (pair_order != nullptr) p = pair_order[p];
        const PairAt at = pair_where(p, pair_list, cell_begin, P.n);
        const uint32_t cell = at.cell, piece = at.piece;
        PairRec rec;
        memset(&rec, 0, sizeof(rec));
        bool skip = outside != nullptr && outside[piece] != 0;
        const uint32_t f0 = plane_off[cell], F = plane_off[cell + 1] - f0;
        if (F > SURTR_MAXF) { rec.status = SURTR_E_INVALID; skip = true; }
        if (!skip)
        {
            int err = SC_FALLBACK;
            uint32_t voff = 0, n = 0, hoff = 0, nh = 0;
            if (P.cdup[piece] == 0)
            {
                for (uint32_t k = tid; k < F; k += group_size()) sh.planes[k] = planes[f0 + k];
                __syncthreads();
                uint32_t which = 0;
                err = small_clip(convex_solid_in(P, piece), F, sh, U.f, &which);
                if (err == 0)
                {
                    const uint32_t nv = U.f.nv[which];
                    if (nv != 0u) err = sc_park(U.f.buf[which], nv, sh, A.cursors, A.pos, A.loff, A.llen, A.nbr, A.capV, A.capH, voff, n, hoff, nh);
                }
                __syncthreads();
            }
            if (err != 0)
            {
                if (tid == 0) giveup[atomicAdd(&A.cursors[CUR_CVX_GAVE_UP], 1u)] = p;
                continue;
            }
            if (tid == 0) atomicAdd(&A.cursors[CUR_CVX_TOOK], 1u);
            rec.cv_off = voff; rec.cv_n = n; rec.ch_off = hoff; rec.ch_n = nh;
        }
        convex_publish(pairs, p, rec, front_par);
        if (rec.cv_n != 0 && porder != nullptr) convex_enqueue_prep(P, piece, p, F, sh.planes, U.pmar, A, porder, n_pairs);
    }
}

#ifndef SURTR_PREP_MINV
#define SURTR_PREP_MINV 2048u
#endif
#ifndef SURTR_PREP_NB
#define SURTR_PREP_NB 1024u
#endif
#ifndef SURTR_PREP_WAVES
#define SURTR_PREP_WAVES 7
#endif
template <bool OLD_SELECT = true>
__device__ __attribute__((always_inline)) static inline void prep_pairs_body(Shared& sh, unsigned long long* lmask, uint2* lblk, uint32_t rec_on,
                                                         const Pieces& P, const float4* __restrict__ planes,
                                                         const uint32_t* __restrict__ plane_off, uint32_t cell_begin,
                                                         uint32_t n_pairs, const PrepPool& pool, const Arena& A, const ImgArena& IA, uint32_t capV, uint32_t capVs,
                                                         PairRec* __restrict__ pairs, const uint2* __restrict__ pair_list,
                                                         uint32_t* __restrict__ order, const uint32_t* __restrict__ porder,
                                                         uint32_t* __restrict__ horder, uint32_t half_on, uint32_t big_quota, uint32_t big_n)
{
    auto enqueue = [&](uint32_t p, uint32_t cls) { order[(size_t)cls * n_pairs + atomicAdd(&A.cursors[CUR_CLS_CLIP + cls], 1u)] = p; };
    auto enqueue_half = [&](uint32_t p, uint32_t cls) { horder[(size_t)cls * n_pairs + atomicAdd(&A.cursors[CUR_CLS_HALF + cls], 1u)] = p; };
    const uint32_t tid = threadIdx.x;
    const bool front_par = (rec_on & 4u) != 0u;
    char* sp = pool.base + (size_t)blockIdx.x * pool.per_wg;
    auto take = [&](size_t bytes) { char* r = sp; sp += (bytes + 255) & ~(size_t)255; return r; };
    uint32_t* needy = (uint32_t*)take((size_t)pool.VMAX * 4);
    uint32_t* orig = (uint32_t*)take((size_t)pool.VMAX * 4);
    uint32_t* und = (uint32_t*)take((size_t)(pool.VMAX / SURTR_SB + 2) * 4);
    unsigned long long* gmask = (unsigned long long*)take((size_t)(pool.VMAX / SURTR_LANES + 2) * 8);
    uint2* gblk = (uint2*)take((size_t)(pool.VMAX / SURTR_LANES + 2) * 8);
    uint8_t* vfc = (uint8_t*)take((size_t)pool.VMAX + 64);
    uint8_t* fcb = (uint8_t*)take((size_t)pool.VMAX + 64);
    uint32_t* klist = (uint32_t*)take((size_t)pool.VMAX * 4);
    uint32_t* walks = (uint32_t*)take((size_t)pool.VMAX * 4);
    uint16_t* sid16 = (uint16_t*)take((size_t)pool.VMAX * 2 + 64);
#ifdef SURTR_STAMP
    const unsigned long long wg_t0 = __builtin_readcyclecounter();
    unsigned long long wg_work = 0;
#endif
    while (true)
    {
        __syncthreads();
        if (tid == 0)
        {
            uint32_t t = atomicAdd(&A.cursors[CUR_Q_PREP], 1u);
            if (front_par) sh.misc[7] = t < n_pairs ? t : 0xFFFFFFFFu;
            else sh.misc[7] = pair_of_ticket(A, porder, n_pairs, t, CUR_CLS_PREP, 15, 0);
        }
        __syncthreads();
        const uint32_t p = sh.misc[7];
        if (p >= n_pairs) break;
        const PairAt at = pair_where(p, pair_list, cell_begin, P.n);
        const uint32_t cell = at.cell, piece = at.piece;
        if (front_par)
        {
            if (tid == 0) { pairs[p].img_fmt = IMG_NONE; pairs[p].img_off = 0; pairs[p].img_n = 0; pairs[p].img_h = 0; pairs[p].img_pc = 0; }
            if (plane_off[cell + 1] - plane_off[cell] > SURTR_MAXF) continue;
        }
        else if (pairs[p].cv_n == 0 || pairs[p].status != 0) continue;
        const uint32_t m0 = P.mvo[piece], V = P.mvo[piece + 1] - m0;
        if (V < SURTR_PREP_MINV || V > pool.VMAX)
        {
            if (tid == 0)
            {
// ... 2587 lines not shown
        rc = ctx->img_buf.grow(ctx, (size_t)cap16 * 16);
        if (rc) return rc;
        ctx->img = ImgArena{ctx->img_buf, cap16};
    }
    return SURTR_OK;
}

static void free_arena(surtr_ctx* ctx)
{
    auto& B = ctx->arena_buf;
    B.pos.reset(); B.loff.reset(); B.llen.reset(); B.nbr.reset(); B.idx.reset(); B.isl.reset();
    ctx->d_frags.reset(); ctx->d_forder.reset(); ctx->d_frag_status.reset(); ctx->d_face_list.reset();
    ctx->arena = Arena{}; ctx->arena.cursors = B.cursors; ctx->cap_frags = 0;
}

static uint32_t refit_planes(const surtr_ctx* ctx) { return std::min(2u * RH_MAXFACE, 2u * (3u * ctx->refit_limit - 8u)); }

static int ensure_arena(surtr_ctx* ctx, uint32_t n_pairs, uint64_t min_v = 0, uint64_t min_h = 0, uint64_t min_i = 0)
{
    const uint64_t xp = refit_planes(ctx) - 8u;
    uint64_t av = ctx->user_av ? ctx->user_av : std::max<uint64_t>(std::max<uint64_t>((uint64_t)ctx->vmax * 8, ctx->tot_mv * 3) + (uint64_t)n_pairs * (256 + 8 * xp), 1u << 16);
    uint64_t ah = ctx->user_ah ? ctx->user_ah : std::max<uint64_t>(std::max<uint64_t>((uint64_t)ctx->hmax * 8, ctx->tot_mh * 3) + (uint64_t)n_pairs * (1024 + 32 * xp), 1u << 18);
    uint64_t ai = ctx->user_ai ? ctx->user_ai : ah * 2;
    av = std::max(av, min_v); ah = std::max(ah, min_h); ai = std::max(ai, min_i);
    av = std::min<uint64_t>(av, 0xFFFFFFF0ull); ah = std::min<uint64_t>(ah, 0xFFFFFFF0ull); ai = std::min<uint64_t>(ai, 0xFFFFFFF0ull);
    const uint32_t capIsl = (uint32_t)std::min<uint64_t>((uint64_t)n_pairs * 4 + 1024, 0x7FFFFFFFull);
    if (!(ctx->arena.pos && ctx->arena.capV >= av && ctx->arena.capH >= ah && ctx->arena.capI >= ai && ctx->arena.capIsl >= capIsl))
    {
        free_arena(ctx);
        auto& B = ctx->arena_buf;
        int rc = B.pos.grow(ctx, av * 3);
        if (rc == SURTR_OK) rc = B.loff.grow(ctx, av);
        if (rc == SURTR_OK) rc = B.llen.grow(ctx, av);
        if (rc == SURTR_OK) rc = B.nbr.grow(ctx, ah);
        if (rc == SURTR_OK) rc = B.idx.grow(ctx, ai);
        if (rc == SURTR_OK) rc = B.isl.grow(ctx, capIsl);
        if (rc == SURTR_OK) rc = ctx->d_frags.grow(ctx, capIsl);
        if (rc == SURTR_OK) rc = ctx->d_forder.grow(ctx, (size_t)capIsl * 16);
        if (rc == SURTR_OK) rc = ctx->d_frag_status.grow(ctx, capIsl);
        if (rc == SURTR_OK) rc = ctx->d_face_list.grow(ctx, capIsl);
        if (rc) { free_arena(ctx); return rc; }
        ctx->arena = Arena{B.pos, B.loff, B.llen, B.nbr, B.idx, B.isl, (uint32_t)av, (uint32_t)ah, (uint32_t)ai, capIsl, B.cursors};
        ctx->cap_frags = capIsl;
    }
    int rc = ctx->d_pairs.grow(ctx, n_pairs);
    if (rc == SURTR_OK) rc = ctx->d_cvx_giveup.grow(ctx, n_pairs);
    if (rc) return rc;
    return ctx->d_scanblk.grow(ctx, std::max(n_pairs, ctx->cap_frags) / SURTR_LANES + 4);
}

__global__ void k_event_init(uint32_t* __restrict__ cursors, uint32_t* __restrict__ counts, uint32_t n_counts, uint32_t* __restrict__ frag_status,
                             uint32_t n_status, uint32_t* __restrict__ hlist, uint32_t n_hlist)
{
    const uint32_t i0 = blockIdx.x * blockDim.x + threadIdx.x, step = gridDim.x * blockDim.x;
    for (uint32_t i = i0; i < CUR_COUNT; i += step) cursors[i] = 0u;
    for (uint32_t i = i0; i < n_counts; i += step) counts[i] = 0u;
    for (uint32_t i = i0; i < n_status; i += step) frag_status[i] = 0u;
    for (uint32_t i = i0; i < n_hlist; i += step) hlist[i] = 0xFFFFFFFFu;
}

static int upload_pair_order(surtr_ctx* ctx, const uint32_t* ord, uint32_t n_pairs)
{
    const int rc = ctx->d_pair_order.grow(ctx, n_pairs);
    if (rc) return rc;
    HIPCHK(hipStreamSynchronize(ctx->stream));
    HIPCHK(hipMemcpyAsync(ctx->d_pair_order, ord, (size_t)n_pairs * 4, hipMemcpyHostToDevice, ctx->stream));
    HIPCHK(hipStreamSynchronize(ctx->stream));
    return SURTR_OK;
}

#ifndef SURTR_REC_MAXN
#define SURTR_REC_MAXN 2304u
#endif
#ifndef SURTR_FRONT_PAR_MAX
#define SURTR_FRONT_PAR_MAX 1024u
#endif
struct EventPlan
{
    bool cell_order;
    decltype(&k_prep_pairs) prep;
    uint32_t prep_threads;
    bool wave_on, split_on, use_half, front_par, both;
    bool cvx_lean;
    uint32_t rec_on;
    uint32_t big_quota, big_n, walk0, n_catch, n_poll;
    uint32_t n_wg, n_wg_cvx, n_wg_lean, n_wg_cvx2, n_wg_prep, n_wg_big, n_wg_half, n_wg_retry, n_wg_sweep;
    uint32_t g_refit, g_faces, t_faces;
    hipStream_t st_cvx, st_main, st_bigk, st_refit;
};

static EventPlan plan_event(const surtr_ctx* ctx, uint32_t n_pairs, bool pair_list, uint32_t flags)
{
    EventPlan pl{};
    const uint32_t n1 = std::max(n_pairs, 1u), max_wg = ctx->max_wg;
    pl.cell_order = !pair_list && n_pairs && ctx->n_pieces && n_pairs % ctx->n_pieces == 0 && !getenv("SURTR_NO_CELL_ORDER");
    pl.n_wg = std::max(1u, std::min(n1, max_wg));
    pl.n_wg_cvx = std::max(1u, std::min(n1, ctx->max_wg_small));
    pl.n_wg_lean = std::max(1u, std::min(n1, ctx->max_wg_lean));
    pl.n_wg_cvx2 = std::min(n1, 64u);
    pl.n_wg_half = std::max(1u, std::min(n1, ctx->max_wg_half));
    pl.n_wg_prep = std::max(1u, std::min(n1, ctx->max_wg_prep));
    pl.n_wg_big = std::min(ctx->n_wg_big, n1);
    pl.n_wg_retry = std::min(pl.n_wg, 64u);
    pl.big_quota = ctx->wave_big ? 0xFFFFFFFFu : 2u * ctx->n_wg_big;
    if (const char* e = getenv("SURTR_BIG_QUOTA")) pl.big_quota = (uint32_t)atoi(e);
    pl.big_n = (ctx->wave_big && ctx->vmax < 180000u) ? 2800u : 0xFFFFFFFFu;
    const bool half_forced = getenv("SURTR_HALF") != nullptr && atoi(getenv("SURTR_HALF")) != 0;
    const bool many = ctx->events_in_flight > 1u && !half_forced;
    pl.wave_on = 2u * n_pairs > 3u * max_wg || (!half_forced && ctx->vmin >= SURTR_PREP_MINV && ctx->vmax <= 4u * SURTR_REC_MAXN) ||
                 (many && ctx->vmin >= SURTR_PREP_MINV && ctx->vmax <= ctx->prep.VMAX);
    if (const char* e = getenv("SURTR_WAVE")) pl.wave_on = atoi(e) != 0;
    pl.rec_on = pl.wave_on ? 1u : 0u;
    if (const char* e = getenv("SURTR_REC")) pl.rec_on = (pl.wave_on && atoi(e) != 0) ? 1u : 0u;
    if (const char* e = getenv("SURTR_PREP_SORTED")) { if (atoi(e) == 0) pl.rec_on = 2u; }
    uint32_t rec_maxn = SURTR_REC_MAXN;
    if (const char* e = getenv("SURTR_REC_MAXN")) rec_maxn = (uint32_t)atoi(e);
    pl.rec_on |= (rec_maxn < 0xFFFFFFu ? rec_maxn : 0xFFFFFFu) << 8;
    pl.split_on = pl.wave_on && ctx->vmin >= SURTR_PREP_MINV && ctx->vmax <= ctx->prep.VMAX;
    if (const char* e = getenv("SURTR_SPLIT")) pl.split_on = pl.split_on && atoi(e) != 0;
    pl.use_half = ctx->half_on && (!pl.split_on || half_forced);
    pl.n_catch = std::min(SURTR_CATCH_WG_MAX, n1);
    pl.n_wg_sweep = std::min(pl.n_catch, SURTR_CATCH_POLL);
    pl.n_poll = ctx->events_in_flight > 1u ? 2u : SURTR_CATCH_POLL;
    if (const char* e = getenv("SURTR_CATCH_POLL")) { const int v = atoi(e); if (v >= 0 && v <= 1024) pl.n_poll = (uint32_t)v; }
    uint32_t wide_max = 4u * ctx->max_wg;
    if (const char* e = getenv("SURTR_PREP_WIDE_MAX")) wide_max = (uint32_t)atoi(e);
    const bool prep_wide = n_pairs != 0 && n_pairs <= wide_max && ctx->vmax >= 8192u && !many;
    pl.front_par = n_pairs != 0 && n_pairs <= SURTR_FRONT_PAR_MAX && !prep_wide;
    if (const char* e = getenv("SURTR_FRONT_PAR")) pl.front_par = n_pairs != 0 && atoi(e) != 0;
    if (pl.front_par) pl.rec_on |= 4u;
    pl.cvx_lean = n_pairs > ctx->max_wg_small;
    if (const char* e = getenv("SURTR_CVX_LEAN")) pl.cvx_lean = n_pairs != 0 && atoi(e) != 0;
    pl.prep = nullptr; pl.prep_threads = SURTR_WG;
    if (n_pairs && prep_wide) { pl.prep = k_prep_pairs_wide; pl.prep_threads = SURTR_WG_WIDE; }
    else if (n_pairs && !(pl.rec_on & 2u) && ctx->vmax < 0xFFFFu && ctx->vmin >= SURTR_PREP_MINV && (ctx->vmax + SURTR_LANES - 1u) / SURTR_LANES <= SURTR_PREP_NB)
        pl.prep = k_prep_pairs_sorted;
    else if (n_pairs) pl.prep = k_prep_pairs;
    pl.walk0 = SURTR_WWALK0;
    if (const char* e = getenv("SURTR_WWALK0")) { const int v = atoi(e); if (v >= 0 && v <= 64) pl.walk0 = (uint32_t)v; }
    pl.st_cvx = pl.front_par ? ctx->stream3 : ctx->stream;
    pl.st_main = pl.front_par ? ctx->stream : ctx->stream2;
    pl.st_bigk = pl.front_par ? ctx->stream2 : ctx->stream;
    pl.both = (flags & SURTR_EVT_REFIT) && (flags & SURTR_EVT_RENDER);
    pl.st_refit = pl.both ? ctx->stream2 : ctx->stream;
    pl.g_refit = ctx->n_wg_small;
    if (pl.both) pl.g_refit = std::min(pl.g_refit, ctx->max_wg_faces / 4u * 5u);
    if (pl.both) if (const char* e = getenv("SURTR_REFIT_WG_BOTH")) { const uint32_t v = (uint32_t)atoi(e); if (v > 0 && v <= ctx->n_wg_small) pl.g_refit = v; }
    pl.g_faces = std::max(1u, ctx->max_wg_faces); pl.t_faces = SURTR_WG;
    if (pl.both) pl.g_faces = std::max(1u, ctx->max_wg_faces / 2u);
    if (pl.both) if (const char* e = getenv("SURTR_FACES_WG_BOTH")) { const uint32_t v = (uint32_t)atoi(e); if (v > 0 && v <= ctx->n_wg_faces_alloc) pl.g_faces = v; }
    if (const char* e = getenv("SURTR_FACES_WG")) { const uint32_t v = (uint32_t)atoi(e); if (v > 0 && v <= ctx->n_wg_faces_alloc) pl.g_faces = v; }
    if (const char* e = getenv("SURTR_FACES_THREADS")) { const uint32_t v = (uint32_t)atoi(e); if (v == 64 || v == 128 || v == 256) pl.t_faces = v; }
    return pl;
}

static int ensure_hull_ws(surtr_ctx* ctx)
{
    if (ctx->refit_limit <= 4u || ctx->d_hull_ws.cap >= 2 * (size_t)ctx->arena.capV) return SURTR_OK;
    HIPCHK(hipStreamSynchronize(ctx->stream));
    return ctx->d_hull_ws.grow(ctx, 2 * (size_t)ctx->arena.capV);
}

static void launch_refit(surtr_ctx* ctx, uint32_t grid, hipStream_t st, bool of_pieces)
{
    const float* cpos = of_pieces ? (const float*)ctx->cset.pos : (const float*)nullptr;
    const uint32_t* cvo = of_pieces ? (const uint32_t*)ctx->cset.vo : (const uint32_t*)nullptr;
    if (ctx->refit_limit <= 4u)
        hipLaunchKernelGGL(k_refit, dim3(grid), dim3(SURTR_LANES), 0, st, ctx->d_frags, ctx->d_counts, ctx->pool_small, ctx->arena, ctx->d_forder, ctx->cap_frags, ctx->d_frag_status,
                           cpos, cvo);
    else
        hipLaunchKernelGGL(k_refit_n, dim3(grid), dim3(SURTR_LANES), 0, st, ctx->d_frags, ctx->d_counts, ctx->pool_small, ctx->arena, ctx->d_forder, ctx->cap_frags, ctx->d_frag_status,
                           cpos, cvo, ctx->refit_limit, (uint32_t*)ctx->d_hull_ws);
}

static int launch_event(surtr_ctx* ctx, uint32_t cell_begin, uint32_t n_pairs, const uint2* d_pair_list, const uint8_t* outside, uint32_t flags)
{
    (void)hipSetDevice(ctx->device);
    budget_workgroups(ctx);
    const uint32_t max_wg = ctx->max_wg, n1 = std::max(n_pairs, 1u);
    int rc = ensure_scratch(ctx, ctx->vmax, ctx->hmax, max_wg + ctx->n_wg_big + SURTR_CATCH_WG_MAX);
    if (rc) return rc;
    rc = ensure_scratch_small(ctx, std::max(ctx->max_wg_small, ctx->n_wg_small));
    if (rc) return rc;
    rc = ensure_scratch_half(ctx, std::max(ctx->max_wg_half, ctx->n_wg_half));
    if (rc) return rc;
    rc = ensure_arena(ctx, n1);
    if (rc) return rc;
    if (flags & SURTR_EVT_REFIT) { rc = ensure_hull_ws(ctx); if (rc) return rc; }
    rc = ensure_prep(ctx, n1, std::max(std::max(1u, std::min(n1, ctx->max_wg_prep)), ctx->n_wg_prep));
    if (rc) return rc;
    hipStream_t st = ctx->stream, st2 = ctx->stream2, st3 = ctx->stream3;
    const uint32_t hcap = n_pairs + 4096u;
    if (ctx->d_hlist.cap < hcap)
    {
        HIPCHK(hipStreamSynchronize(st));
        rc = ctx->d_hlist.grow(ctx, hcap);
        if (rc) return rc;
    }
    const EventPlan pl = plan_event(ctx, n_pairs, d_pair_list != nullptr, flags);
    static_assert(sizeof(surtr_counts) % 4 == 0, "surtr_counts is cleared by words");
    hipLaunchKernelGGL(k_event_init, dim3(SURTR_LANES == 1 ? 1 : 64), dim3(SURTR_LANES == 1 ? 1 : 256), 0, st, ctx->arena.cursors, (uint32_t*)ctx->d_counts.p,
                       (uint32_t)(sizeof(surtr_counts) / 4), ctx->d_frag_status, ctx->cap_frags, ctx->d_hlist, hcap);
    const uint8_t* d_out = nullptr;
    ctx->last_outside.clear();
    if (outside) ctx->last_outside.assign(outside, outside + ctx->n_pieces);
    if (outside)
    {
        HIPCHK(hipMemcpyAsync(ctx->d_outside, outside, ctx->n_pieces, hipMemcpyHostToDevice, st));
        d_out = ctx->d_outside;
    }
    const PieceSet& M = ctx->mset; const PieceSet& C = ctx->cset;
    Pieces P{M.pos, M.loff, M.llen, M.nbr, M.vo, M.tri, M.rad, M.perm, M.posr_s, M.bsph, M.bo,
             C.pos, C.loff, C.llen, C.nbr, C.vo, C.tri, C.rad, C.perm, C.posr_s, C.bsph, C.bo, ctx->n_pieces, M.dup, C.dup,
             M.row_s, M.iperm, M.bsph2, M.bo2, M.bsph3, M.bo3};
    for (int i = 0; i < 16; ++i) ctx->ev_valid[i] = false;
    const uint32_t* d_pair_order = nullptr;
    if (d_pair_list && ctx->pair_order_is_list && ctx->pair_order_count == n_pairs) d_pair_order = ctx->d_pair_order;
    else if (pl.cell_order)
    {
        const uint32_t np = ctx->n_pieces, nc = n_pairs / np;
        if (ctx->pair_order_is_list || ctx->pair_order_begin != cell_begin || ctx->pair_order_count != n_pairs)
        {
            std::vector<uint32_t> cells(nc), ord((size_t)n_pairs);
            for (uint32_t i = 0; i < nc; ++i) cells[i] = i;
            const std::vector<uint32_t>& po = ctx->h_plane_off;
            std::stable_sort(cells.begin(), cells.end(), [&](uint32_t a, uint32_t b) {
                return po[cell_begin + a + 1] - po[cell_begin + a] > po[cell_begin + b + 1] - po[cell_begin + b]; });
            for (uint32_t i = 0; i < nc; ++i) for (uint32_t q = 0; q < np; ++q) ord[(size_t)i * np + q] = cells[i] * np + q;
            int rc2 = upload_pair_order(ctx, ord.data(), n_pairs);
            if (rc2) return rc2;
            ctx->pair_order_is_list = false; ctx->pair_order_begin = cell_begin; ctx->pair_order_count = n_pairs;
        }
        d_pair_order = ctx->d_pair_order;
    }
    uint32_t* const order = ctx->d_order;
    const size_t cap_order = ctx->d_order.cap / 64;
    uint32_t* const porder = ctx->d_order + 16 * cap_order;
    uint32_t* const horder = ctx->d_order + 32 * cap_order;
    const bool wave = n_pairs && pl.wave_on, split = wave && pl.split_on;

    if (pl.front_par)
    {
        HIPCHK(hipEventRecord(ctx->ev_prep, st));
        HIPCHK(hipStreamWaitEvent(pl.st_cvx, ctx->ev_prep, 0));
    }
    PROF_BEGIN_ON(6, pl.st_cvx);
    if (n_pairs && pl.cvx_lean)
    {
        uint32_t* const cvx_porder = pl.front_par ? (uint32_t*)nullptr : porder;
        hipLaunchKernelGGL(k_clip_convex_lean, dim3(pl.n_wg_lean), dim3(SURTR_LANES), 0, pl.st_cvx, P, ctx->d_planes, ctx->d_plane_off, cell_begin, n_pairs,
                           d_out, ctx->arena, ctx->d_pairs, d_pair_list, cvx_porder, d_pair_order, pl.front_par ? 1u : 0u, (uint32_t*)ctx->d_cvx_giveup);
        hipLaunchKernelGGL(k_clip_convex, dim3(pl.n_wg_cvx2), dim3(SURTR_LANES), 0, pl.st_cvx, P, ctx->d_planes, ctx->d_plane_off, cell_begin, n_pairs,
                           d_out, ctx->pool_small, ctx->arena, ctx->d_pairs, d_pair_list, cvx_porder, (const uint32_t*)nullptr,
                           pl.front_par ? 1u : 0u, (const uint32_t*)ctx->d_cvx_giveup);
    }
    else if (n_pairs)
        hipLaunchKernelGGL(k_clip_convex, dim3(pl.n_wg_cvx), dim3(SURTR_LANES), 0, pl.st_cvx, P, ctx->d_planes, ctx->d_plane_off, cell_begin, n_pairs,
                           d_out, ctx->pool_small, ctx->arena, ctx->d_pairs, d_pair_list, pl.front_par ? (uint32_t*)nullptr : porder, d_pair_order,
                           pl.front_par ? 1u : 0u, (const uint32_t*)nullptr);
    PROF_END_ON(6, pl.st_cvx);
    if (pl.front_par) HIPCHK(hipEventRecord(ctx->ev_cvx, pl.st_cvx));
    PROF_BEGIN(7);
    if (pl.prep)
        hipLaunchKernelGGL(pl.prep, dim3(pl.n_wg_prep), dim3(pl.prep_threads), 0, st, P, ctx->d_planes, ctx->d_plane_off, cell_begin, n_pairs,
                           ctx->prep, ctx->arena, ctx->img, std::min((uint32_t)SURTR_LV, ctx->pool.CV), std::min((uint32_t)SURTR_LVS, ctx->pool_half.CV),
                           ctx->d_pairs, d_pair_list, order, porder, horder, pl.use_half ? 1u : 0u, pl.big_quota, pl.big_n, pl.rec_on);
    PROF_END(7);
    HIPCHK(hipEventRecord(ctx->ev_prep, st));
    HIPCHK(hipStreamWaitEvent(st2, ctx->ev_prep, 0));
    HIPCHK(hipStreamWaitEvent(st3, ctx->ev_prep, 0));
    if (pl.front_par)
    {
        HIPCHK(hipStreamWaitEvent(st, ctx->ev_cvx, 0));
        HIPCHK(hipStreamWaitEvent(st2, ctx->ev_cvx, 0));
    }
    PROF_BEGIN_ON(8, pl.st_bigk);
    if (n_pairs && ctx->wave_big)
        hipLaunchKernelGGL(k_clip_pairs_wave_big, dim3(pl.n_wg_big), dim3(SURTR_WG), 0, pl.st_bigk, P, ctx->d_planes,
                           ctx->d_plane_off, cell_begin, n_pairs, ctx->pool, max_wg, ctx->arena, ctx->img, ctx->d_pairs, d_pair_list, order, 15, 14, CUR_Q_BIG, pl.walk0);
    else if (n_pairs)
        hipLaunchKernelGGL(k_clip_pairs_big, dim3(pl.n_wg_big), dim3(SURTR_WG), 0, pl.st_bigk, P, ctx->d_planes,
                           ctx->d_plane_off, cell_begin, n_pairs, ctx->pool, max_wg, ctx->arena, ctx->img, ctx->d_pairs, d_pair_list, order);
    PROF_END_ON(8, pl.st_bigk);
    PROF_BEGIN_ON(11, pl.st_main);
    if (wave) PROF_HIST_BEGIN(11, pl.st_main);
    if (split)
        hipLaunchKernelGGL(k_clip_pairs_main, dim3(pl.n_wg), dim3(SURTR_MAIN_THREADS), 0, pl.st_main, P, ctx->d_planes, ctx->d_plane_off, cell_begin, n_pairs,
                           ctx->pool, ctx->arena, ctx->img, ctx->d_pairs, d_pair_list, order, ctx->d_hlist, pl.walk0);
    else if (wave)
        hipLaunchKernelGGL(k_clip_pairs_wave, dim3(pl.n_wg), dim3(SURTR_WG), 0, pl.st_main, P, ctx->d_planes, ctx->d_plane_off, cell_begin, n_pairs,
                           ctx->pool, ctx->arena, ctx->img, ctx->d_pairs, d_pair_list, order, horder, 13, 0, CUR_Q_CLIP, pl.walk0);
    if (wave) PROF_HIST_END(11, pl.st_main);
    PROF_END_ON(11, pl.st_main);
    PROF_BEGIN_ON(0, pl.st_main);
    if (n_pairs && !pl.wave_on)
    {
        PROF_HIST_BEGIN(0, pl.st_main);
// ... 474 lines not shown
int surtr_debug_stamps(unsigned long long out[96], int reset)
{
    if (hipMemcpyFromSymbol(out, HIP_SYMBOL(g_stamp), sizeof(unsigned long long) * 96) != hipSuccess) return SURTR_E_HIP;
    if (reset) { unsigned long long z[96] = {}; (void)hipMemcpyToSymbol(HIP_SYMBOL(g_stamp), z, sizeof(z)); }
    return SURTR_OK;
}
#endif

int surtr_set_events_in_flight(surtr_ctx* ctx, uint32_t n)
{
    if (!ctx) return SURTR_E_INVALID;
    ctx->events_in_flight = n ? n : 1u;
    return SURTR_OK;
}

int surtr_set_profiling(surtr_ctx* ctx, int on)
{
    if (!ctx) return SURTR_E_INVALID;
    (void)hipSetDevice(ctx->device);
    if (on && !ctx->ev[0])
        for (int i = 0; i < 32; ++i) HIPCHK(hipEventCreate(&ctx->ev[i]));
    if (on && !ctx->hev[0][0])
        for (int i = 0; i < 16; ++i) { HIPCHK(hipEventCreate(&ctx->hev[i][0])); HIPCHK(hipEventCreate(&ctx->hev[i][1])); }
    ctx->hcount = 0;
    ctx->profiling = on != 0;
    return SURTR_OK;
}

int surtr_kernel_times(surtr_ctx* ctx, float ms[16])
{
    if (!ctx || !ms) return SURTR_E_INVALID;
    for (int i = 0; i < 16; ++i) ms[i] = -1.f;
    (void)hipSetDevice(ctx->device);
    HIPCHK(hipStreamSynchronize(ctx->stream));
    for (int i = 0; i < 16; ++i)
        if (ctx->ev_valid[i]) { float t = 0.f; if (hipEventElapsedTime(&t, ctx->ev[2 * i], ctx->ev[2 * i + 1]) == hipSuccess) ms[i] = t; }
    return SURTR_OK;
}

int surtr_kernel_history(surtr_ctx* ctx, float ms[16], int slot[16], uint32_t* n)
{
    if (!ctx || !ms || !slot || !n) return SURTR_E_INVALID;
    (void)hipSetDevice(ctx->device);
    HIPCHK(hipStreamSynchronize(ctx->stream));
    const uint32_t have = ctx->hcount < 16u ? ctx->hcount : 16u;
    for (uint32_t k = 0; k < have; ++k)
    {
        const uint32_t at = (ctx->hcount - have + k) % 16u;
        float t = -1.f;
        if (hipEventElapsedTime(&t, ctx->hev[at][0], ctx->hev[at][1]) != hipSuccess) t = -1.f;
        ms[k] = t; slot[k] = ctx->hslot[at];
    }
    *n = have;
    return SURTR_OK;
}

int surtr_pair_status(surtr_ctx* ctx, uint32_t n_pairs, uint32_t* status)
{
    if (!ctx || !status) return SURTR_E_INVALID;
    if (!ctx->have_event || n_pairs > ctx->d_pairs.cap) return SURTR_E_STATE;
    (void)hipSetDevice(ctx->device);
    HIPCHK(hipStreamSynchronize(ctx->stream));
    std::vector<PairRec> recs(n_pairs);
    if (n_pairs) HIPCHK(hipMemcpy(recs.data(), ctx->d_pairs, (size_t)n_pairs * sizeof(PairRec), hipMemcpyDeviceToHost));
    for (uint32_t i = 0; i < n_pairs; ++i) status[i] = recs[i].status;
    return SURTR_OK;
}

int surtr_event_pair_costs(surtr_ctx* ctx, uint32_t n_pairs, uint32_t* cost)
{
    if (!ctx || !cost) return SURTR_E_INVALID;
    if (!ctx->have_event || n_pairs > ctx->d_pairs.cap) return SURTR_E_STATE;
    (void)hipSetDevice(ctx->device);
    HIPCHK(hipStreamSynchronize(ctx->stream));
    std::vector<PairRec> recs(n_pairs);
    if (n_pairs) HIPCHK(hipMemcpy(recs.data(), ctx->d_pairs, (size_t)n_pairs * sizeof(PairRec), hipMemcpyDeviceToHost));
    for (uint32_t i = 0; i < n_pairs; ++i)
    {
        const PairRec& r = recs[i];
        uint32_t c = 8u;
        if (r.cv_n != 0) c += (r.img_fmt == IMG_NARROW || r.img_fmt == IMG_WIDE ? r.img_n : 256u) + 4u * r.mv_n + 64u;
        cost[i] = c;
    }
    return SURTR_OK;
}

int surtr_set_refit_point_limit(surtr_ctx* ctx, uint32_t n)
{
    if (!ctx || n < 4u || n > RH_MAXPT) return SURTR_E_INVALID;
    ctx->refit_limit = n;
    return SURTR_OK;
}

int surtr_get_refit_point_limit(surtr_ctx* ctx, uint32_t* n)
{
    if (!ctx || !n) return SURTR_E_INVALID;
    *n = ctx->refit_limit;
    return SURTR_OK;
}

int surtr_coord_key(float x, uint32_t* neg, uint64_t* scaled)
{
    if (!neg || !scaled) return SURTR_E_INVALID;
    return rh_coord_key(x, scaled, neg) ? SURTR_OK : SURTR_E_CAPACITY;
}

int surtr_hull_normals_device(surtr_ctx* ctx, uint32_t n, const float* points, uint32_t limit, uint32_t capacity, float* normals, uint32_t* count)
{
    if (!ctx || !points || !count || n < 4u || limit < 4u || limit > RH_MAXPT) return SURTR_E_INVALID;
    (void)hipSetDevice(ctx->device);
    DevBuf<float> d_pts, d_nrm; DevBuf<uint32_t> d_ws, d_out;
    if (d_pts.grow(ctx, 3 * (size_t)n) || d_nrm.grow(ctx, 3 * RH_MAXFACE) || d_ws.grow(ctx, 2 * (size_t)n) || d_out.grow(ctx, 2)) return SURTR_E_HIP;
    hipStream_t st = ctx->stream;
    HIPCHK(hipMemcpyAsync(d_pts, points, (size_t)n * 12, hipMemcpyHostToDevice, st));
    hipLaunchKernelGGL(k_hull_probe, dim3(1), dim3(SURTR_LANES), 0, st, (const float*)d_pts, n, limit, (uint32_t*)d_ws, (float*)d_nrm, (uint32_t*)d_out);
    HIPCHK(hipGetLastError());
    HIPCHK(hipStreamSynchronize(st));
    uint32_t out[2] = {0u, 0u};
    HIPCHK(hipMemcpy(out, d_out, 8, hipMemcpyDeviceToHost));
    if (out[0] != 0u) return (int)out[0];
    *count = out[1];
    if (!normals) return SURTR_OK;
    if (out[1] > capacity) return SURTR_E_CAPACITY;
    if (out[1]) HIPCHK(hipMemcpy(normals, d_nrm, (size_t)out[1] * 12, hipMemcpyDeviceToHost));
    return SURTR_OK;
}

int surtr_queue_stats(surtr_ctx* ctx, uint32_t out[128])
{
    if (!ctx || !out) return SURTR_E_INVALID;
    (void)hipSetDevice(ctx->device);
    HIPCHK(hipStreamSynchronize(ctx->stream));
    HIPCHK(hipMemcpy(out, ctx->arena.cursors, CUR_STATS_WORDS * 4, hipMemcpyDeviceToHost));
    return SURTR_OK;
}

int surtr_blob_unpack_host(const void* blob, size_t bytes, surtr_counts* counts, surtr_fragments* out)
{
    if (!blob || bytes < 64) return SURTR_E_INVALID;
    surtr_counts c;
    memcpy(&c, blob, sizeof(c));
    const BlobLayout L = blob_layout(c);
    if (L.total > bytes) return SURTR_E_CAPACITY;
    if (counts) *counts = c;
    if (!out) return SURTR_OK;
    const char* b = (const char*)blob;
    auto cp = [&](void* dst, size_t off, size_t n) { if (dst && n) memcpy(dst, b + off, n); };
    cp(out->frag_ids, L.ids, (size_t)c.n_frag * 12);
    cp(out->mesh_vert_off, L.mvo, ((size_t)c.n_frag + 1) * 4);
    cp(out->mesh_pos, L.mpos, (size_t)c.mesh_verts * 12);
    cp(out->mesh_nbr_off, L.mno, ((size_t)c.mesh_verts + 1) * 4);
    cp(out->mesh_nbr, L.mnbr, (size_t)c.mesh_nbrs * 4);
    cp(out->conv_vert_off, L.cvo, ((size_t)c.n_frag + 1) * 4);
    cp(out->conv_pos, L.cpos, (size_t)c.conv_verts * 12);
    cp(out->conv_nbr_off, L.cno, ((size_t)c.conv_verts + 1) * 4);
    cp(out->conv_nbr, L.cnbr, (size_t)c.conv_nbrs * 4);
    cp(out->vnc, L.vnc, (size_t)c.mesh_verts * 36);
    cp(out->idx_off, L.ioff, ((size_t)c.n_frag + 1) * 4);
    cp(out->idx, L.idx, (size_t)c.n_idx * 4);
    cp(out->frag_status, L.fstat, (size_t)c.n_frag * 4);
    return SURTR_OK;
}

int surtr_event_download(surtr_ctx* ctx, surtr_fragments* out)
{
    if (!ctx || !out) return SURTR_E_INVALID;
// ... 61 lines not shown
```

surtr_amd/engine.py:

```python
import ctypes
import os

import numpy as np

_HERE = os.path.dirname(os.path.abspath(__file__))
_LIB = None

OK, E_INVALID, E_TOPOLOGY, E_CAPACITY, E_HIP, E_STATE, E_NOGPU = range(7)
EVT_REFIT, EVT_RENDER = 1, 2
CELLS_ALL = 0xFFFFFFFF


class SurtrError(RuntimeError):
    def __init__(self, code, msg=""):
        self.code = code
        RuntimeError.__init__(self, "surtr error %d: %s %s" % (code, _strerror(code), msg))


class Counts(ctypes.Structure):
    _fields_ = [(n, ctypes.c_uint32) for n in
                ("n_frag", "mesh_verts", "mesh_nbrs", "conv_verts", "conv_nbrs", "n_idx", "n_pairs", "status", "n_failed")]


class Mass(ctypes.Structure):
    _fields_ = [("volume", ctypes.c_double), ("mass", ctypes.c_double), ("com", ctypes.c_double * 3),
                ("inertia", ctypes.c_double * 6), ("nv", ctypes.c_uint32), ("status", ctypes.c_uint32)]


MASS_DTYPE = np.dtype([("volume", "<f8"), ("mass", "<f8"), ("com", "<f8", (3,)), ("inertia", "<f8", (6,)),
                       ("nv", "<u4"), ("status", "<u4")])
assert MASS_DTYPE.itemsize == ctypes.sizeof(Mass) == 96

HULL_DTYPE = np.dtype([("nv", "<u4"), ("n_faces", "<u4"), ("n_idx", "<u4"), ("status", "<u4"), ("face_off", "<u4"), ("idx_off", "<u4"),
                       ("max_loop", "<u4"), ("reserved0", "<u4"), ("convexity", "<f4"), ("planarity", "<f4"), ("extent", "<f4"),
                       ("reserved1", "<u4")])
POLY_DTYPE = np.dtype([("plane", "<f4", (4,)), ("n_verts", "<u2"), ("index_base", "<u2")])
assert HULL_DTYPE.itemsize == 48 and POLY_DTYPE.itemsize == 20
HULL_FEW, HULL_OPEN, HULL_FLAT, HULL_IRREGULAR, HULL_LARGE, HULL_OVER_255 = 1, 2, 4, 8, 16, 32
HULL_WITHHELD = HULL_FEW | HULL_OPEN | HULL_IRREGULAR | HULL_LARGE


def hull_usable(record, rel_tol=1e-5):
    if int(record["status"]) & (HULL_WITHHELD | HULL_FLAT):
        return False
    tol = np.float32(rel_tol) * np.float32(record["extent"])
    return bool(record["convexity"] <= tol and record["planarity"] <= tol)


SHADED_DTYPE = np.dtype([("first_vertex", "<u4"), ("n_vertices", "<u4"), ("n_faces", "<u4"), ("status", "<u4")])
assert SHADED_DTYPE.itemsize == 16
SHADE_PER_TRIANGLE = 1
SHADE_NO_FACE = 0xFFFFFFFF


COOK_DTYPE = np.dtype([("nv_in", "<u4"), ("nv", "<u4"), ("n_faces", "<u4"), ("n_idx", "<u4"), ("status", "<u4"), ("pt_off", "<u4"),
                       ("face_off", "<u4"), ("idx_off", "<u4"), ("max_loop", "<u4"), ("n_welded", "<u4"), ("convexity", "<f4"),
                       ("planarity", "<f4"), ("extent", "<f4"), ("reach", "<f4"), ("reserved", "<u4", (2,))])
assert COOK_DTYPE.itemsize == 64
COOK_SKIPPED, COOK_FEW, COOK_DEGENERATE, COOK_NONFINITE, COOK_LARGE, COOK_FAILED, COOK_OVER_255 = 1, 2, 4, 8, 16, 32, 64
COOK_WITHHELD = COOK_SKIPPED | COOK_FEW | COOK_DEGENERATE | COOK_NONFINITE | COOK_LARGE | COOK_FAILED


def cooked_usable(record, plane_tol=7e-6, weld_dist=0.0):
    if int(record["status"]) & COOK_WITHHELD:
        return False
    s = 2.0 ** -24 * 3.5 * float(record["reach"])
    return bool(record["planarity"] <= plane_tol + s and record["convexity"] <= 2.0 * plane_tol + weld_dist + s)


def cook_max_vertices():
    f = lib().surtr_cook_max_vertices
    f.restype = ctypes.c_uint32
    return int(f())


RAY_HIT_DTYPE = np.dtype([("piece", "<i4"), ("status", "<u4"), ("t", "<f4"), ("pos", "<f4", (3,)), ("normal", "<f4", (3,)),
                          ("reserved", "<u4", (3,))])
assert RAY_HIT_DTYPE.itemsize == 48
SCENE_RAY_HIT_DTYPE = np.dtype([("piece", "<i4"), ("status", "<u4"), ("t", "<f4"), ("pos", "<f4", (3,)), ("normal", "<f4", (3,)),
                                ("compound", "<i4"), ("reserved", "<u4", (2,))])
assert SCENE_RAY_HIT_DTYPE.itemsize == 48
RAY_STARTS_INSIDE, RAY_INVALID = 1, 2
QUERY_FEW, QUERY_OPEN, QUERY_FLAT, QUERY_LONG = 1, 2, 4, 8
BOUNDS_DTYPE = np.dtype([("lo", "<f4", (3,)), ("hi", "<f4", (3,)), ("n_vertices", "<u4"), ("status", "<u4")])
assert BOUNDS_DTYPE.itemsize == 32
BOUNDS_NONFINITE = 1
CULL_LIGHT, CULL_OUTSIDE = 1, 2


_DERIVED = (("llen", np.uint32), ("tri", np.uint8), ("rad", np.float32), ("box", np.float32), ("perm", np.uint32),
            ("posr_s", np.float32), ("bsph", np.float32), ("bsph2", np.float32), ("bsph3", np.float32), ("iperm", np.uint32),
            ("row_s", np.uint16), ("dup", np.uint8), ("bo", np.uint32), ("bo2", np.uint32), ("bo3", np.uint32), ("build", np.uint32))


class Fragments(ctypes.Structure):
    _fields_ = [(n, ctypes.c_void_p) for n in
                ("frag_ids", "mesh_vert_off", "mesh_pos", "mesh_nbr_off", "mesh_nbr", "conv_vert_off", "conv_pos",
                 "conv_nbr_off", "conv_nbr", "vnc", "idx_off", "idx", "frag_status")]


def lib_path():
    return os.path.join(_HERE, "libsurtr_hip.so")


def _configure(L):
    L.surtr_strerror.restype = ctypes.c_char_p
    L.surtr_last_error.restype = ctypes.c_char_p
    L.surtr_last_error.argtypes = [ctypes.c_void_p]
    L.surtr_event_blob_bytes.restype = ctypes.c_size_t
    L.surtr_destroy.argtypes = [ctypes.c_void_p]
    L.surtr_destroy.restype = None
    return L


def _use_library_for_tests(path):
    global _LIB
    _LIB = _configure(ctypes.CDLL(path)) if path else None


def _share_hip_runtime_with_torch():
    import sys, importlib.util
    if "torch" in sys.modules:
        return
    try:
        spec = importlib.util.find_spec("torch")
    except (ImportError, ValueError):
        spec = None
    if spec is None or not spec.submodule_search_locations:
        return
    cand = os.path.join(list(spec.submodule_search_locations)[0], "lib", "libamdhip64.so")
    if os.path.exists(cand):
        try:
            ctypes.CDLL(cand, mode=ctypes.RTLD_GLOBAL)
        except OSError:
            pass


def lib():
    global _LIB
    if _LIB is None:
        if not os.path.exists(lib_path()):
            raise ImportError("libsurtr_hip.so is not built: run `python -c 'import __graft_entry__ as g; g.build()'`")
        _share_hip_runtime_with_torch()
        L = _configure(ctypes.CDLL(lib_path()))
        _LIB = L
    return _LIB


def _strerror(code):
    try:
        return lib().surtr_strerror(ctypes.c_int(code)).decode()
    except Exception:
        return "?"


def _p(a):
    return None if a is None else a.ctypes.data_as(ctypes.c_void_p)


def _solid_arrays(s):
    return (np.ascontiguousarray(s["pos"], np.float32).reshape(-1, 3), np.ascontiguousarray(s["off"], np.uint32),
            np.ascontiguousarray(s["nbr"], np.int32))


def pack_solids(solids):
    vo = [0]
    pos, off, nbr = [], [np.zeros(1, np.int64)], []
    base = 0
    for s in solids:
        p = np.ascontiguousarray(s["pos"], np.float32).reshape(-1, 3)
        o = np.asarray(s["off"], np.int64)
        pos.append(p)
        off.append(o[1:] + base)
        base += int(o[-1])
        nbr.append(np.asarray(s["nbr"], np.int32))
# ... 8 lines not shown
    to[1:] = np.cumsum([x.shape[0] for x in lists])
    return to, (np.concatenate(lists) if lists else np.zeros(0, np.uint32)).astype(np.uint32)


def _impact_spheres(sphere_points, origins, radii, k=None):
    if origins is not None:
        k = np.ascontiguousarray(origins, np.float32).reshape(-1, 3).shape[0]
    k = int(k or 0)
    org = np.zeros((k, 3), np.float32) if origins is None else np.ascontiguousarray(origins, np.float32).reshape(-1, 3)
    rad = np.zeros(k, np.float32) if radii is None else np.ascontiguousarray(radii, np.float32).reshape(-1)
    clouds = [np.zeros((0, 3), np.float32)] * k if sphere_points is None else \
        [np.zeros((0, 3), np.float32) if c is None else np.ascontiguousarray(c, np.float32).reshape(-1, 3) for c in sphere_points]
    if not len(clouds) == org.shape[0] == rad.shape[0] == k:
        raise SurtrError(E_INVALID, "one cloud, origin and radius per impact")
    so = np.zeros(k + 1, np.uint32)
    so[1:] = np.cumsum([c.shape[0] for c in clouds])
    sp = np.ascontiguousarray(np.concatenate(clouds) if clouds else np.zeros((0, 3), np.float32), np.float32)
    if sp.shape[0] == 0:
        sp = np.zeros((1, 3), np.float32)
    return k, so, sp, org, rad


class Engine:

    def __init__(self, device=0, stream=None):
        self._h = ctypes.c_void_p()
        rc = lib().surtr_create(ctypes.c_int(device), ctypes.byref(self._h))
        if rc:
            raise SurtrError(rc)
        if stream is not None:
            self.set_stream(stream)

    def close(self):
        if self._h:
            lib().surtr_destroy(self._h)
            self._h = ctypes.c_void_p()

    def __del__(self):
        try:
            self.close()
        except Exception:
            pass

    def _ck(self, rc):
        if rc:
            raise SurtrError(rc, lib().surtr_last_error(self._h).decode())

    def set_stream(self, stream_ptr):
        self._ck(lib().surtr_set_stream(self._h, ctypes.c_void_p(stream_ptr)))

    def set_scratch(self, max_verts, max_nbrs):
        self._ck(lib().surtr_set_scratch(self._h, ctypes.c_uint32(max_verts), ctypes.c_uint32(max_nbrs)))

    def set_arena(self, verts, nbrs, idx):
        self._ck(lib().surtr_set_arena(self._h, ctypes.c_uint64(verts), ctypes.c_uint64(nbrs), ctypes.c_uint64(idx)))

    def set_profiling(self, on=True):
        self._ck(lib().surtr_set_profiling(self._h, ctypes.c_int(int(on))))

    def kernel_times(self):
        ms = (ctypes.c_float * 16)()
        self._ck(lib().surtr_kernel_times(self._h, ms))
        names = ("clip_pairs", "frag_table", "refit", "faces", "out_scan", "pack", "clip_convex", "prep_pairs", "clip_pairs_big", "clip_pairs_half", "clip_pairs_retry", "clip_pairs_wave", None, "clip_pairs_catch")
        return {n: float(ms[i]) for i, n in enumerate(names) if n}

    def set_events_in_flight(self, n):
        self._ck(lib().surtr_set_events_in_flight(self._h, ctypes.c_uint32(int(n))))

    def kernel_history(self):
        ms = (ctypes.c_float * 16)(); slot = (ctypes.c_int * 16)(); n = ctypes.c_uint32(0)
        self._ck(lib().surtr_kernel_history(self._h, ms, slot, ctypes.byref(n)))
        return [float(ms[i]) for i in range(n.value)]

    def pair_status(self, n_pairs):
        out = np.zeros(n_pairs, dtype=np.uint32)
        self._ck(lib().surtr_pair_status(self._h, ctypes.c_uint32(n_pairs), _p(out)))
        return out

    def pair_costs(self, n_pairs):
        out = np.zeros(n_pairs, dtype=np.uint32)
        self._ck(lib().surtr_event_pair_costs(self._h, ctypes.c_uint32(n_pairs), _p(out)))
        return out

    def queue_stats(self):
        out = (ctypes.c_uint32 * 128)()
        self._ck(lib().surtr_queue_stats(self._h, out))
        return np.frombuffer(out, dtype=np.uint32).copy()

    def handover_stats(self):
        out = (ctypes.c_uint32 * 8)()
        self._ck(lib().surtr_handover_stats(self._h, out))
        names = ("pushed", "main_started", "main_signed_off", "poll_claimed", "catch_own", "sweep_cursor", "max_wg", "hcap")
        return {n: int(out[i]) for i, n in enumerate(names)}

    def pair_order(self):
        n = ctypes.c_uint32()
        self._ck(lib().surtr_pair_order(self._h, ctypes.c_uint32(0), ctypes.byref(n), None))
        out = np.zeros(n.value, np.uint32)
        self._ck(lib().surtr_pair_order(self._h, ctypes.c_uint32(n.value), ctypes.byref(n), _p(out)))
        return out

    def upload_pieces(self, meshes, convexes):
        assert len(meshes) == len(convexes)
        m = pack_solids(meshes)
        c = pack_solids(convexes)
        self._ck(lib().surtr_upload_pieces(self._h, ctypes.c_uint32(len(meshes)), _p(m[0]), _p(m[1]), _p(m[2]), _p(m[3]),
                                           _p(c[0]), _p(c[1]), _p(c[2]), _p(c[3])))

    def build_cells(self, seeds, group_seed_off=None):
        s = np.ascontiguousarray(seeds, np.float64).reshape(-1, 3)
        go = np.array([0, s.shape[0]], np.uint32) if group_seed_off is None else np.ascontiguousarray(group_seed_off, np.uint32)
        nf, nfv = ctypes.c_uint32(), ctypes.c_uint32()
        self._ck(lib().surtr_build_cells(self._h, ctypes.c_uint32(go.shape[0] - 1), _p(go), _p(s), ctypes.byref(nf), ctypes.byref(nfv)))
        self._cells_n = (s.shape[0], nf.value, nfv.value)
        return nf.value, nfv.value

    def download_cells(self):
        n, nf, nfv = self._cells_n
        cfo = np.zeros(n + 1, np.uint32); gen = np.zeros(nf, np.int32); fvo = np.zeros(nf + 1, np.uint32)
        verts = np.zeros((nfv, 3), np.float64); v012 = np.zeros((nf, 9), np.float32)
        self._ck(lib().surtr_download_cells(self._h, _p(cfo), _p(gen), _p(fvo), _p(verts), _p(v012)))
        return {"cell_face_off": cfo, "face_gen": gen, "face_vert_off": fvo, "verts": verts, "v012": v012}

    def neighbors_from_mesh(self, pos, tris):
        pos = np.ascontiguousarray(pos, np.float32).reshape(-1, 3)
        tris = np.ascontiguousarray(tris, np.int32).reshape(-1, 3)
        off = np.zeros(pos.shape[0] + 1, np.uint32)
        nbr = np.zeros(3 * tris.shape[0] + 4, np.int32)
        ms = ctypes.c_float()
        self._ck(lib().surtr_neighbors_from_mesh_dev(self._h, ctypes.c_uint32(pos.shape[0]), ctypes.c_uint32(tris.shape[0]), _p(tris), _p(off), _p(nbr),
                                                     ctypes.byref(ms)))
        return {"pos": pos, "off": off, "nbr": nbr[:off[-1]].copy()}, float(ms.value)

    def upload_pattern(self, face_off, v012):
        fo = np.ascontiguousarray(face_off, np.uint32)
        v = np.ascontiguousarray(v012, np.float32).reshape(-1, 9)
        assert v.shape[0] == fo[-1]
        self._ck(lib().surtr_upload_pattern(self._h, ctypes.c_uint32(fo.shape[0] - 1), _p(fo), _p(v)))

    def place_cells(self, scale, translate):
        s = np.ascontiguousarray(scale, np.float32)
        t = np.ascontiguousarray(translate, np.float32)
        self._ck(lib().surtr_place_cells(self._h, _p(s), _p(t)))

    def place_cells_impacts(self, scales, translates):
        s = np.ascontiguousarray(scales, np.float32).reshape(-1, 3)
        t = np.ascontiguousarray(translates, np.float32).reshape(-1, 3)
        if s.shape[0] != t.shape[0]:
            raise SurtrError(E_INVALID, "%d scales, %d translates" % (s.shape[0], t.shape[0]))
        self._ck(lib().surtr_place_cells_impacts(self._h, ctypes.c_uint32(s.shape[0]), _p(s), _p(t)))

    def pattern_store(self):
        i = ctypes.c_uint32()
        self._ck(lib().surtr_pattern_store(self._h, ctypes.byref(i)))
        return i.value

    def pattern_count(self):
        n = ctypes.c_uint32()
        self._ck(lib().surtr_pattern_count(self._h, ctypes.byref(n)))
        return n.value

    def pattern_info(self, id):
        nc, nf = ctypes.c_uint32(), ctypes.c_uint32()
        self._ck(lib().surtr_pattern_info(self._h, ctypes.c_uint32(int(id)), ctypes.byref(nc), ctypes.byref(nf)))
        return nc.value, nf.value

# ... 177 lines not shown

    def _cook_sel(self, fn, hulls, rel_tol, weld_dist, plane_tol):
        h = None if hulls is None else np.ascontiguousarray(hulls, HULL_DTYPE)
        return self._cook(lambda *a: fn(self._h, None if h is None else _p(h), ctypes.c_uint32(0 if h is None else h.shape[0]),
                                        ctypes.c_float(rel_tol), ctypes.c_float(weld_dist), ctypes.c_float(plane_tol), *a))

    def event_cook(self, hulls=None, rel_tol=1e-5, weld_dist=0.0, plane_tol=7e-6):
        return self._cook_sel(lib().surtr_event_cook, hulls, rel_tol, weld_dist, plane_tol)

    def pieces_cook(self, hulls=None, rel_tol=1e-5, weld_dist=0.0, plane_tol=7e-6):
        return self._cook_sel(lib().surtr_pieces_cook, hulls, rel_tol, weld_dist, plane_tol)

    def cook_points(self, solids, weld_dist=0.0, plane_tol=7e-6):
        arrs = [np.ascontiguousarray(a, np.float32).reshape(-1, 3) for a in solids]
        vo = np.concatenate([[0], np.cumsum([a.shape[0] for a in arrs])]).astype(np.uint32)
        pos = np.ascontiguousarray(np.concatenate(arrs) if arrs else np.zeros((0, 3), np.float32), np.float32)
        return self._cook(lambda *a: lib().surtr_cook_points(self._h, ctypes.c_uint32(len(arrs)), _p(vo), _p(pos), ctypes.c_float(weld_dist),
                                                             ctypes.c_float(plane_tol), *a))

    def _cook_dev(self, fn, dev_hulls, rel_tol, weld_dist, plane_tol, dev_records, records_bytes, dev_points, points_cap, dev_src, dev_polys,
                  polys_cap, dev_idx, idx_cap):
        self._ck(fn(self._h, ctypes.c_void_p(dev_hulls or None), ctypes.c_float(rel_tol), ctypes.c_float(weld_dist), ctypes.c_float(plane_tol),
                    ctypes.c_void_p(dev_records), ctypes.c_size_t(records_bytes), ctypes.c_void_p(dev_points), ctypes.c_size_t(points_cap),
                    ctypes.c_void_p(dev_src), ctypes.c_void_p(dev_polys), ctypes.c_size_t(polys_cap), ctypes.c_void_p(dev_idx), ctypes.c_size_t(idx_cap)))

    def event_cook_dev(self, dev_hulls, rel_tol, weld_dist, plane_tol, dev_records, records_bytes, dev_points, points_cap, dev_src, dev_polys,
                       polys_cap, dev_idx, idx_cap):
        self._cook_dev(lib().surtr_event_cook_dev, dev_hulls, rel_tol, weld_dist, plane_tol, dev_records, records_bytes, dev_points, points_cap,
                       dev_src, dev_polys, polys_cap, dev_idx, idx_cap)

    def pieces_cook_dev(self, dev_hulls, rel_tol, weld_dist, plane_tol, dev_records, records_bytes, dev_points, points_cap, dev_src, dev_polys,
                        polys_cap, dev_idx, idx_cap):
        self._cook_dev(lib().surtr_pieces_cook_dev, dev_hulls, rel_tol, weld_dist, plane_tol, dev_records, records_bytes, dev_points, points_cap,
                       dev_src, dev_polys, polys_cap, dev_idx, idx_cap)

    def pieces_raycast(self, rays):
        r = np.ascontiguousarray(rays, np.float32).reshape(-1, 7)
        out = np.zeros(r.shape[0], RAY_HIT_DTYPE)
        self._ck(lib().surtr_pieces_raycast(self._h, ctypes.c_uint32(r.shape[0]), _p(r), _p(out)))
        return out

    def pieces_overlap(self, spheres, mass=None, min_mass=1e-4):
        sp = np.ascontiguousarray(spheres, np.float32).reshape(-1, 4)
        m = None if mass is None else np.ascontiguousarray(mass, MASS_DTYPE)
        n = ctypes.c_uint32()
        args = [self._h, ctypes.c_uint32(sp.shape[0]), _p(sp), _p(m), ctypes.c_float(min_mass)]
        self._ck(lib().surtr_pieces_overlap(*args, ctypes.byref(n), None))
        if m is not None and m.shape[0] != n.value:
            raise SurtrError(E_INVALID, "mass holds %d records for %d pieces" % (m.shape[0], n.value))
        out = np.zeros((sp.shape[0], n.value), np.uint8)
        self._ck(lib().surtr_pieces_overlap(*args, ctypes.byref(n), _p(out)))
        return out

    def pieces_raycast_dev(self, n_rays, dev_rays, dev_hits, capacity):
        self._ck(lib().surtr_pieces_raycast_dev(self._h, ctypes.c_uint32(int(n_rays)), ctypes.c_void_p(dev_rays), ctypes.c_void_p(dev_hits),
                                                ctypes.c_size_t(capacity)))

    def pieces_overlap_dev(self, n_spheres, dev_spheres, dev_mask, capacity, dev_mass=None, min_mass=1e-4):
        self._ck(lib().surtr_pieces_overlap_dev(self._h, ctypes.c_uint32(int(n_spheres)), ctypes.c_void_p(dev_spheres),
                                                ctypes.c_void_p(dev_mass), ctypes.c_float(min_mass), ctypes.c_void_p(dev_mask),
                                                ctypes.c_size_t(capacity)))

    def pieces_query_status(self, n):
        out = np.zeros(int(n), np.uint32)
        self._ck(lib().surtr_pieces_query_status(self._h, ctypes.c_uint32(int(n)), _p(out)))
        return out

    def download_piece(self, piece, set=1):
        nv, nh = ctypes.c_uint32(), ctypes.c_uint32()
        args = [self._h, ctypes.c_uint32(int(piece)), ctypes.c_int(int(set))]
        self._ck(lib().surtr_download_piece(*args, ctypes.byref(nv), ctypes.byref(nh), None, None, None))
        pos = np.zeros((nv.value, 3), np.float32); off = np.zeros(nv.value + 1, np.uint32); nbr = np.zeros(nh.value, np.int32)
        self._ck(lib().surtr_download_piece(*args, ctypes.byref(nv), ctypes.byref(nh), _p(pos), _p(off), _p(nbr)))
        return {"pos": pos, "off": off, "nbr": nbr}

    def pieces_derived(self, set=0):
        def get(which, dtype):
            b = ctypes.c_size_t()
            args = [self._h, ctypes.c_int(int(set)), ctypes.c_int(which)]
            self._ck(lib().surtr_pieces_derived(*args, None, ctypes.c_size_t(0), ctypes.byref(b)))
            buf = np.zeros(b.value, np.uint8)
            self._ck(lib().surtr_pieces_derived(*args, _p(buf), ctypes.c_size_t(b.value), ctypes.byref(b)))
            return buf.view(dtype)
        out = {name: get(which, dt) for which, (name, dt) in enumerate(_DERIVED)}
        for name, width in (("box", 6), ("posr_s", 4), ("bsph", 4), ("bsph2", 4), ("bsph3", 4), ("row_s", 8)):
            out[name] = out[name].reshape(-1, width)
        build = out.pop("build")
        out["SB"], out["FAN"] = int(build[0]), int(build[1])
        return out

    def event_refit(self):
        self._ck(lib().surtr_event_refit(self._h))

    def set_refit_point_limit(self, n):
        self._ck(lib().surtr_set_refit_point_limit(self._h, ctypes.c_uint32(int(n))))

    def get_refit_point_limit(self):
        n = ctypes.c_uint32()
        self._ck(lib().surtr_get_refit_point_limit(self._h, ctypes.byref(n)))
        return int(n.value)

    def hull_normals_device(self, points, limit):
        p = np.ascontiguousarray(points, np.float32).reshape(-1, 3)
        cnt = ctypes.c_uint32()
        out = np.zeros((63, 3), np.float32)
        self._ck(lib().surtr_hull_normals_device(self._h, ctypes.c_uint32(p.shape[0]), _p(p), ctypes.c_uint32(int(limit)), ctypes.c_uint32(63),
                                                 _p(out), ctypes.byref(cnt)))
        return out[:cnt.value].copy()

    def event_counts(self):
        c = Counts()
        self._ck(lib().surtr_event_counts(self._h, ctypes.byref(c)))
        return c

    def pack_dev(self, dev_ptr, capacity):
        self._ck(lib().surtr_event_pack_dev(self._h, ctypes.c_void_p(dev_ptr), ctypes.c_size_t(capacity)))

    def download(self):
        c = self.event_counts()
        out = alloc_fragments(c)
        fr = _frag_struct(out)
        self._ck(lib().surtr_event_download(self._h, ctypes.byref(fr)))
        return shape_fragments(out)

    def load_fragments(self, meshes, convexes, frag_ids=None):
        m = pack_solids(meshes)
        c = pack_solids(convexes)
        ids = None if frag_ids is None else np.ascontiguousarray(frag_ids, np.int32)
        self._ck(lib().surtr_load_fragments(self._h, ctypes.c_uint32(len(meshes)), _p(m[0]), _p(m[1]), _p(m[2]), _p(m[3]),
                                            _p(c[0]), _p(c[1]), _p(c[2]), _p(c[3]), _p(ids)))

    def event_triangulate(self, is_convex=False):
        self._ck(lib().surtr_event_triangulate(self._h, ctypes.c_int(int(is_convex))))

    def refit_solid(self, mesh, convex):
        mp, mo, mn = _solid_arrays(mesh)
        cp, co, cn = _solid_arrays(convex)
        nv, nh = ctypes.c_uint32(), ctypes.c_uint32()
        args = [self._h, ctypes.c_uint32(mp.shape[0]), _p(mp), _p(mo), _p(mn), ctypes.c_uint32(cp.shape[0]), _p(cp), _p(co), _p(cn)]
        self._ck(lib().surtr_refit_solid(*args, ctypes.byref(nv), ctypes.byref(nh), None, None, None))
        opos = np.zeros((nv.value, 3), np.float32); ooff = np.zeros(nv.value + 1, np.uint32); onbr = np.zeros(nh.value, np.int32)
        self._ck(lib().surtr_refit_solid(*args, ctypes.byref(nv), ctypes.byref(nh), _p(opos), _p(ooff), _p(onbr)))
        return {"pos": opos, "off": ooff, "nbr": onbr}

    def extract_faces(self, solid):
        p, o, n = _solid_arrays(solid)
        nf, ni = ctypes.c_uint32(), ctypes.c_uint32()
        args = [self._h, ctypes.c_uint32(p.shape[0]), _p(p), _p(o), _p(n)]
        self._ck(lib().surtr_extract_faces(*args, ctypes.byref(nf), ctypes.byref(ni), None, None))
        fo = np.zeros(nf.value + 1, np.uint32); fi = np.zeros(ni.value, np.int32)
        self._ck(lib().surtr_extract_faces(*args, ctypes.byref(nf), ctypes.byref(ni), _p(fo), _p(fi)))
        return fo, fi

    def triangulate(self, solid, is_convex=False, color=None):
        p, o, n = _solid_arrays(solid)
        col = None if color is None else np.ascontiguousarray(color, np.float32)
        ni = ctypes.c_uint32()
        args = [self._h, ctypes.c_uint32(p.shape[0]), _p(p), _p(o), _p(n), ctypes.c_int(int(is_convex)), _p(col)]
        self._ck(lib().surtr_triangulate(*args, None, ctypes.byref(ni), None))
        vnc = np.zeros((p.shape[0], 9), np.float32); idx = np.zeros(ni.value, np.uint32)
        self._ck(lib().surtr_triangulate(*args, _p(vnc), ctypes.byref(ni), _p(idx)))
        return vnc, idx

    def transform_pieces(self, world):
        w = np.ascontiguousarray(world, np.float32).reshape(-1, 16)
        self._ck(lib().surtr_transform_pieces(self._h, ctypes.c_uint32(w.shape[0]), _p(w)))

    def pieces_from_event(self, keep=None):
        k = None if keep is None else np.ascontiguousarray(keep, np.uint8)
        n = ctypes.c_uint32()
        self._ck(lib().surtr_pieces_from_event(self._h, _p(k), ctypes.byref(n)))
        return n.value
# ... 512 lines not shown
```

Before: 1.258 million.

## Precompute convex piece adjacency images at upload and bulk-copy them in small_clip

Adds a kernel, run when convex pieces are uploaded, that builds packed vertex-word and reverse-edge tables plus a per-piece validity flag. At event time small_clip copies these tables into LDS with vectorized 16-byte loads instead of rebuilding adjacency and searching for reverse edges per pair, which removes the per-pair validation and ring scans. The cost is extra device memory, extra upload work, and a second code path that has to match the old encoding. The feature is on by default and can be turned off with an environment variable; it also adds probe and debug APIs.

Result: no change. 1.258 million (median of 2 runs) (-0.0%).

```diff
diff --git a/include/surtr_hip.h b/include/surtr_hip.h
--- a/include/surtr_hip.h
+++ b/include/surtr_hip.h
@@ -67,6 +67,7 @@
 int surtr_queue_stats(surtr_ctx* ctx, uint32_t out[128]);
 int surtr_pair_status(surtr_ctx* ctx, uint32_t n_pairs, uint32_t* status);
 int surtr_event_pair_costs(surtr_ctx* ctx, uint32_t n_pairs, uint32_t* cost);
+int surtr_prep_queue(surtr_ctx* ctx, uint32_t n_pairs, uint32_t* n, uint32_t* pairs);
 
 int surtr_upload_pieces(surtr_ctx* ctx, uint32_t n_pieces,
                         const uint32_t* mesh_vert_off, const float* mesh_pos,
@@ -153,9 +154,14 @@
     SURTR_DERIVED_BO2 = 13,
     SURTR_DERIVED_BO3 = 14,
     SURTR_DERIVED_BUILD = 15,
-    SURTR_DERIVED_COUNT = 16
+    SURTR_DERIVED_IMG_VW = 16,
+    SURTR_DERIVED_IMG_RE = 17,
+    SURTR_DERIVED_IMG_REG = 18,
+    SURTR_DERIVED_COUNT = 19
 };
 int surtr_pieces_derived(surtr_ctx* ctx, int set, int which, void* out, size_t capacity_bytes, size_t* bytes);
+int surtr_convex_image_probe(surtr_ctx* ctx, uint32_t n, const uint32_t* vo, const uint32_t* off, const int32_t* nbr, uint32_t* vw,
+                             uint32_t* re, uint8_t* reg);
 int surtr_upload_stats(surtr_ctx* ctx, float* ms, uint32_t* n_alloc);
 int surtr_handover_stats(surtr_ctx* ctx, uint32_t out[8]);
 int surtr_regroup_stats(surtr_ctx* ctx, uint32_t out[8]);
diff --git a/surtr_amd/csrc/pieces_dev.hip b/surtr_amd/csrc/pieces_dev.hip
--- a/surtr_amd/csrc/pieces_dev.hip
+++ b/surtr_amd/csrc/pieces_dev.hip
@@ -46,6 +46,32 @@
         for (uint32_t q = ulo; q < uhi && q >= ulo; ++q) if (nbr[q] == lv) { back = true; break; }
         if (!back) { atomicMax(err, (uint32_t)SURTR_E_TOPOLOGY); return; }
     }
+}
+
+__global__ void k_piece_image(uint32_t V, uint32_t n, const uint32_t* __restrict__ vo, const uint32_t* __restrict__ loff,
+                              const int32_t* __restrict__ nbr, const uint32_t* __restrict__ gate, uint32_t* __restrict__ vw,
+                              uint32_t* __restrict__ re, uint8_t* __restrict__ reg)
+{
+    const uint32_t v = blockIdx.x * blockDim.x + threadIdx.x;
+    if (v >= V) return;
+    if (gate && *gate) return;
+    const uint32_t p = piece_of(vo, n, v), a = vo[p], m = vo[p + 1] - a, h0 = loff[a];
+    const uint32_t lo = loff[v], deg = loff[v + 1] - lo;
+    bool odd = deg < 3u || deg > 15u || m > 0xFFFFu || loff[a + m] - h0 > 0xFFFFu;
+    vw[v] = ((lo - h0) & 0xFFFFu) | ((deg & 0xFFFFu) << 16);
+    const uint32_t lv = v - a;
+    for (uint32_t j = 0; j < deg; ++j)
+    {
+        const uint32_t u = (uint32_t)nbr[lo + j];
+        if (u >= m) { odd = true; re[lo + j] = 0; continue; }
+        if (deg <= 15u) for (uint32_t jj = 0; jj < j; ++jj) if ((uint32_t)nbr[lo + jj] == u) odd = true;
+        const uint32_t ulo = loff[a + u], udeg = loff[a + u + 1] - ulo;
+        uint32_t q = 0;
+        while (q < udeg && q < 16u && (uint32_t)nbr[ulo + q] != lv) ++q;
+        if (q >= udeg || q >= 16u) { odd = true; q = 0; }
+        re[lo + j] = u | (q << 16);
+    }
+    if (odd) reg[p] = 0;
 }
 
 __global__ void k_piece_tri_rad(uint32_t V, uint32_t n, const uint32_t* __restrict__ vo, const float* __restrict__ pos,
@@ -288,6 +314,8 @@
         grow_pieces(ctx, S.bsph2, (size_t)NB / SURTR_SPH_FAN + n + 1) || grow_pieces(ctx, S.bo2, n + 1) ||
         grow_pieces(ctx, S.bsph3, (size_t)NB / (SURTR_SPH_FAN * SURTR_SPH_FAN) + n + 1) || grow_pieces(ctx, S.bo3, n + 1))
         return SURTR_E_HIP;
+    if (&S == &ctx->cset && (grow_pieces(ctx, S.img_vw, (size_t)V + 4) || grow_pieces(ctx, S.img_re, (size_t)H + 4) || grow_pieces(ctx, S.reg, n + 1)))
+        return SURTR_E_HIP;
     return SURTR_OK;
 }
 
@@ -301,6 +329,12 @@
     hipLaunchKernelGGL(k_piece_check, gridV, blk, 0, st, V, n, S.vo, S.loff, S.nbr, S.llen, check ? 1u : 0u, ctx->d_upload_err, S.dup, check ? H : 0xFFFFFFFFu);
     hipLaunchKernelGGL(k_piece_tri_rad, gridV, blk, 0, st, V, n, S.vo, S.pos, S.loff, S.nbr, S.tri, S.rad,
                        check ? (const uint32_t*)ctx->d_upload_err.p : (const uint32_t*)nullptr);
+    if (&S == &ctx->cset)
+    {
+        HIPCHK(hipMemsetAsync(S.reg, 1, (size_t)n + 1, st));
+        hipLaunchKernelGGL(k_piece_image, gridV, blk, 0, st, V, n, S.vo, S.loff, S.nbr, check ? (const uint32_t*)ctx->d_upload_err.p : (const uint32_t*)nullptr,
+                           S.img_vw.p, S.img_re.p, S.reg.p);
+    }
     hipLaunchKernelGGL(k_piece_box, dim3(n), dim3(SURTR_WG), 0, st, n, S.vo, S.pos, S.box);
     hipLaunchKernelGGL(k_piece_keys, gridV, blk, 0, st, V, n, S.vo, S.pos, S.box, S.key, S.val);
     int end_bit = 32;
@@ -611,9 +645,35 @@
     return SURTR_OK;
 }
 
+int surtr_convex_image_probe(surtr_ctx* ctx, uint32_t n, const uint32_t* vo, const uint32_t* off, const int32_t* nbr, uint32_t* vw, uint32_t* re, uint8_t* reg)
+{
+    if (!ctx || n == 0 || !vo || !off || !nbr || !vw || !re || !reg || vo[0] != 0) return SURTR_E_INVALID;
+    for (uint32_t p = 0; p < n; ++p) if (vo[p + 1] <= vo[p]) return SURTR_E_INVALID;
+    const uint32_t V = vo[n], H = off[V];
+    for (uint32_t v = 0; v < V; ++v) if (off[v + 1] < off[v] || off[v + 1] > H) return SURTR_E_INVALID;
+    (void)hipSetDevice(ctx->device);
+    hipStream_t st = ctx->stream;
+    DevBuf<uint32_t> d_vo, d_off, d_vw, d_re; DevBuf<int32_t> d_nbr; DevBuf<uint8_t> d_reg;
+    if (d_vo.grow(ctx, n + 1) || d_off.grow(ctx, (size_t)V + 1) || d_nbr.grow(ctx, (size_t)H + 1) || d_vw.grow(ctx, (size_t)V + 4) ||
+        d_re.grow(ctx, (size_t)H + 4) || d_reg.grow(ctx, n + 1))
+        return SURTR_E_HIP;
+    HIPCHK(hipMemcpyAsync(d_vo, vo, (size_t)(n + 1) * 4, hipMemcpyHostToDevice, st));
+    HIPCHK(hipMemcpyAsync(d_off, off, (size_t)(V + 1) * 4, hipMemcpyHostToDevice, st));
+    if (H) HIPCHK(hipMemcpyAsync(d_nbr, nbr, (size_t)H * 4, hipMemcpyHostToDevice, st));
+    HIPCHK(hipMemsetAsync(d_reg, 1, (size_t)n + 1, st));
+    hipLaunchKernelGGL(k_piece_image, dim3((V + 255) / 256), dim3(256), 0, st, V, n, d_vo.p, d_off.p, d_nbr.p, (const uint32_t*)nullptr, d_vw.p, d_re.p, d_reg.p);
+    HIPCHK(hipGetLastError());
+    HIPCHK(hipMemcpyAsync(vw, d_vw, (size_t)V * 4, hipMemcpyDeviceToHost, st));
+    if (H) HIPCHK(hipMemcpyAsync(re, d_re, (size_t)H * 4, hipMemcpyDeviceToHost, st));
+    HIPCHK(hipMemcpyAsync(reg, d_reg, n, hipMemcpyDeviceToHost, st));
+    HIPCHK(hipStreamSynchronize(st));
+    return SURTR_OK;
+}
+
 int surtr_pieces_derived(surtr_ctx* ctx, int set, int which, void* out, size_t capacity_bytes, size_t* bytes)
 {
     if (!ctx || set < 0 || set > 1 || !bytes || which < 0 || which >= SURTR_DERIVED_COUNT) return SURTR_E_INVALID;
+    if (which >= SURTR_DERIVED_IMG_VW && set != 1) return SURTR_E_INVALID;
     const uint32_t build[2] = {SURTR_SB, SURTR_SPH_FAN};
     const void* src = nullptr; size_t b = 0;
     if (which == SURTR_DERIVED_BUILD) b = sizeof(build);
@@ -641,7 +701,10 @@
         case SURTR_DERIVED_DUP:    src = S.dup.p;    b = n; break;
         case SURTR_DERIVED_BO:     src = S.bo.p;     b = ((size_t)n + 1) * 4; break;
         case SURTR_DERIVED_BO2:    src = S.bo2.p;    b = ((size_t)n + 1) * 4; break;
-        default:                   src = S.bo3.p;    b = ((size_t)n + 1) * 4; break;
+        case SURTR_DERIVED_BO3:    src = S.bo3.p;    b = ((size_t)n + 1) * 4; break;
+        case SURTR_DERIVED_IMG_VW: src = S.img_vw.p; b = V * 4; break;
+        case SURTR_DERIVED_IMG_RE: src = S.img_re.p; b = (size_t)ctx->h_ho[set][n] * 4; break;
+        default:                   src = S.reg.p;    b = n; break;
         }
     }
     *bytes = b;
diff --git a/surtr_amd/csrc/small_clip.h b/surtr_amd/csrc/small_clip.h
--- a/surtr_amd/csrc/small_clip.h
+++ b/surtr_amd/csrc/small_clip.h
@@ -38,8 +38,33 @@
 };
 typedef ScLdsT<SC_V, SC_H> ScLds;
 
+struct ScImage { const uint32_t* vw; const uint32_t* re; const float* pos; uint32_t v0, h0; };
+struct alignas(16) ScQuad { uint32_t w[4]; };
+template <uint32_t CAP, class Put>
+__device__ __forceinline__ void sc_copy_quads(const uint32_t* __restrict__ src, size_t first, uint32_t n, Put put)
+{
+    constexpr uint32_t TRIPS = ((CAP + 6u) / 4u + SURTR_LANES - 1u) / SURTR_LANES;
+    const uint32_t skip = (uint32_t)(first & 3u), nq = (skip + n + 3u) >> 2, lane = lane_id();
+    const ScQuad* q = (const ScQuad*)(src + (first - skip));
+    ScQuad r[TRIPS];
+#pragma unroll
+    for (uint32_t t = 0; t < TRIPS; ++t)
+    {
+        const uint32_t i = lane + t * SURTR_LANES;
+        r[t] = i < nq ? q[i] : ScQuad{{0u, 0u, 0u, 0u}};
+    }
+#pragma unroll
+    for (uint32_t t = 0; t < TRIPS; ++t)
+    {
+        const uint32_t i = 4u * (lane + t * SURTR_LANES) - skip;
+#pragma unroll
+        for (uint32_t k = 0; k < 4u; ++k) if (i + k < n) put(i + k, r[t].w[k]);
+    }
+}
+
 template <class SH, class LDS>
-__device__ inline int small_clip(const SolidIn in, const uint32_t F, const SH& sh, LDS& L, uint32_t* which, uint32_t* stop = nullptr)
+__device__ inline int small_clip(const SolidIn in, const uint32_t F, const SH& sh, LDS& L, uint32_t* which, uint32_t* stop = nullptr,
+                                 const ScImage img = ScImage{nullptr, nullptr, nullptr, 0u, 0u})
 {
     typedef typename LDS::Solid ScSolid;
     constexpr uint32_t CAPV = LDS::kV, CAPH = LDS::kH;
@@ -57,42 +82,54 @@
     if (V == 0 || V > CAPV) return SC_FALLBACK;
     const uint32_t hbase = in.loff[0], H = in.loff[V - 1u] + in.llen[V - 1u] - hbase;
     if (H > CAPH) return SC_FALLBACK;
-    bool odd = false;
-    for (uint32_t v = lane; v < V; v += SURTR_LANES)
+    if (img.vw != nullptr)
     {
         ScSolid& S = L.buf[0];
-        S.pos[3 * v] = in.pos[3 * v]; S.pos[3 * v + 1] = in.pos[3 * v + 1]; S.pos[3 * v + 2] = in.pos[3 * v + 2];
-        const uint32_t lo = in.loff[v] - hbase, deg = in.llen[v];
-        if (deg > 15u || deg < 3u) odd = true;
-        const uint32_t dl = deg > 15u ? 15u : deg;
-        S.vw[v] = lo | (dl << VS);
-        const int32_t* r = in.nbr + in.loff[v];
-        for (uint32_t j = 0; j < dl && lo + j < CAPH; ++j)
-        {
-            if ((uint32_t)r[j] >= V) odd = true;
-            S.re[lo + j] = (uint32_t)r[j] & RM;
-            for (uint32_t jj = 0; jj < j; ++jj) if (r[jj] == r[j]) odd = true;
-        }
-    }
-    if (__ballot(odd) != 0ull) return SC_FALLBACK;
-    __syncthreads();
-    for (uint32_t v = lane; v < V; v += SURTR_LANES)
-    {
-        ScSolid& S = L.buf[0];
-        const uint32_t w = S.vw[v], lo = w & VM, deg = w >> VS;
-        for (uint32_t j = 0; j < deg; ++j)
-        {
-            const uint32_t e = S.re[lo + j] & RM;
-            const uint32_t we = S.vw[e], elo = we & VM, edeg = we >> VS;
-            uint32_t q = 0;
-            while (q < edeg && (S.re[elo + q] & RM) != v) ++q;
-            if (q >= edeg) odd = true;
-            S.re[lo + j] = e | (q << RS);
-        }
-    }
-    if (__ballot(odd) != 0ull) return SC_FALLBACK;
-    __syncthreads();
-    SC_STAMP(0);
+        sc_copy_quads<CAPV>(img.vw, img.v0, V, [&](uint32_t i, uint32_t w) { S.vw[i] = (typename ScSolid::Word)((w & 0xFFFFu) | ((w >> 16) << VS)); });
+        sc_copy_quads<CAPH>(img.re, img.h0, H, [&](uint32_t i, uint32_t w) { S.re[i] = (typename ScSolid::Word)((w & 0xFFFFu) | ((w >> 16) << RS)); });
+        sc_copy_quads<3u * CAPV>((const uint32_t*)img.pos, 3u * (size_t)img.v0, 3u * V, [&](uint32_t i, uint32_t w) { S.pos[i] = __uint_as_float(w); });
+        __syncthreads();
+        SC_STAMP(0);
+    }
+    else
+    {
+        bool odd = false;
+        for (uint32_t v = lane; v < V; v += SURTR_LANES)
+        {
+            ScSolid& S = L.buf[0];
+            S.pos[3 * v] = in.pos[3 * v]; S.pos[3 * v + 1] = in.pos[3 * v + 1]; S.pos[3 * v + 2] = in.pos[3 * v + 2];
+            const uint32_t lo = in.loff[v] - hbase, deg = in.llen[v];
+            if (deg > 15u || deg < 3u) odd = true;
+            const uint32_t dl = deg > 15u ? 15u : deg;
+            S.vw[v] = lo | (dl << VS);
+            const int32_t* r = in.nbr + in.loff[v];
+            for (uint32_t j = 0; j < dl && lo + j < CAPH; ++j)
+            {
+                if ((uint32_t)r[j] >= V) odd = true;
+                S.re[lo + j] = (uint32_t)r[j] & RM;
+                for (uint32_t jj = 0; jj < j; ++jj) if (r[jj] == r[j]) odd = true;
+            }
+        }
+        if (__ballot(odd) != 0ull) return SC_FALLBACK;
+        __syncthreads();
+        for (uint32_t v = lane; v < V; v += SURTR_LANES)
+        {
+            ScSolid& S = L.buf[0];
+            const uint32_t w = S.vw[v], lo = w & VM, deg = w >> VS;
+            for (uint32_t j = 0; j < deg; ++j)
+            {
+                const uint32_t e = S.re[lo + j] & RM;
+                const uint32_t we = S.vw[e], elo = we & VM, edeg = we >> VS;
+                uint32_t q = 0;
+                while (q < edeg && (S.re[elo + q] & RM) != v) ++q;
+                if (q >= edeg) odd = true;
+                S.re[lo + j] = e | (q << RS);
+            }
+        }
+        if (__ballot(odd) != 0ull) return SC_FALLBACK;
+        __syncthreads();
+        SC_STAMP(0);
+    }
 #define SC_GIVE_UP do { if (stop != nullptr) { *stop = k; *which = cur; if (lane == 0) L.nv[cur] = nv; __syncthreads(); } return SC_FALLBACK; } while (0)
     uint32_t cur = 0, nv = V;
     for (uint32_t k = 0; k < F && nv != 0u; ++k)
diff --git a/surtr_amd/csrc/surtr_ctx.h b/surtr_amd/csrc/surtr_ctx.h
--- a/surtr_amd/csrc/surtr_ctx.h
+++ b/surtr_amd/csrc/surtr_ctx.h
@@ -136,6 +136,7 @@
     const uint8_t* mdup; const uint8_t* cdup;
     const SRow* mrow_s; const uint32_t* miperm;
     const float4* mbsph2; const uint32_t* mbo2; const float4* mbsph3; const uint32_t* mbo3;
+    const uint32_t* cimg_vw; const uint32_t* cimg_re; const uint8_t* creg;
 };
 
 struct ScratchPool
@@ -221,6 +222,7 @@
     DevBuf<uint8_t> dup;
     DevBuf<uint32_t> iperm; DevBuf<SRow> row_s;
     DevBuf<float4> bsph2; DevBuf<uint32_t> bo2; DevBuf<float4> bsph3; DevBuf<uint32_t> bo3;
+    DevBuf<uint32_t> img_vw, img_re; DevBuf<uint8_t> reg;
 };
 
 struct CellBuffers
diff --git a/surtr_amd/csrc/surtr_hip.hip b/surtr_amd/csrc/surtr_hip.hip
--- a/surtr_amd/csrc/surtr_hip.hip
+++ b/surtr_amd/csrc/surtr_hip.hip
@@ -303,6 +303,12 @@
     const uint32_t c0 = P.cvo[piece];
     return SolidIn{P.cpos + 3 * (size_t)c0, P.cloff + c0, P.cllen + c0, P.cnbr, P.cvo[piece + 1] - c0, P.ctri + c0, P.crad + c0,
                    P.cperm + c0, P.cposr_s + c0, P.cbsph + P.cbo[piece]};
+}
+__device__ __forceinline__ ScImage convex_image(const Pieces& P, uint32_t piece)
+{
+    if (P.cimg_vw == nullptr || P.creg[piece] == 0) return ScImage{nullptr, nullptr, nullptr, 0u, 0u};
+    const uint32_t c0 = P.cvo[piece];
+    return ScImage{P.cimg_vw, P.cimg_re, P.cpos, c0, P.cloff[c0]};
 }
 __device__ __forceinline__ int finish_pair(const Arena& A, PairRec* __restrict__ pairs, uint32_t p, PairRec& rec, int err)
 {
@@ -618,7 +624,8 @@
 struct ChainStamp { unsigned long long t_small, t_park; int path; };
 template <class Literal>
 __device__ __forceinline__ ParkOut convex_chain(const SolidIn cin, const uint32_t F, bool literal_first, const ChainCaller who, Literal&& literal,
-                                                Shared& sh, OneWaveLds& U, Scratch& S, const ScratchPool& pool, const Arena& A, ChainStamp& st)
+                                                Shared& sh, OneWaveLds& U, Scratch& S, const ScratchPool& pool, const Arena& A, ChainStamp& st,
+                                                const ScImage img = ScImage{nullptr, nullptr, nullptr, 0u, 0u})
 {
     const uint32_t tid = threadIdx.x;
     ParkOut o{SURTR_E_TOPOLOGY, 0u, 0u, 0u, 0u, false};
@@ -627,7 +634,7 @@
     literal_first = false;
     o.err = SC_FALLBACK;
 #else
-    if (!literal_first) o.err = small_clip(cin, F, sh, U.f, &which, &stop);
+    if (!literal_first) o.err = small_clip(cin, F, sh, U.f, &which, &stop, img);
 #endif
     if (tid == 0 && (!literal_first || who.count_literal_first)) atomicAdd(&A.cursors[who.slot_took + (o.err == 0 ? 0u : 1u)], 1u);
 #ifdef SURTR_STAMP
@@ -809,7 +816,8 @@
             for (uint32_t k = tid; k < F; k += group_size()) sh.planes[k] = planes[f0 + k];
             __syncthreads();
             const ChainCaller who{CUR_CVX_TOOK, CUR_CVX_RESUMED, true, nullptr, planes + f0};
-            const ParkOut o = convex_chain(convex_solid_in(P, piece), F, P.cdup[piece] != 0, who, [&] { return LiteralArg{convex_solid_in(P, piece), false}; }, sh, U, S, pool, A, cst);
+            const ParkOut o = convex_chain(convex_solid_in(P, piece), F, P.cdup[piece] != 0, who, [&] { return LiteralArg{convex_solid_in(P, piece), false}; }, sh, U, S, pool, A, cst,
+                                           convex_image(P, piece));
             err = o.err; rec.cv_off = o.voff; rec.cv_n = o.n; rec.ch_off = o.hoff; rec.ch_n = o.nh;
         }
         if (err == SURTR_E_TOPOLOGY) { rec.cv_bad = 1; rec.cv_off = 0; rec.cv_n = 1; rec.ch_off = 0; rec.ch_n = 0; err = 0; }
@@ -895,7 +903,7 @@
                 for (uint32_t k = tid; k < F; k += group_size()) sh.planes[k] = planes[f0 + k];
                 __syncthreads();
                 uint32_t which = 0;
-                err = small_clip(convex_solid_in(P, piece), F, sh, U.f, &which);
+                err = small_clip(convex_solid_in(P, piece), F, sh, U.f, &which, nullptr, convex_image(P, piece));
                 if (err == 0)
                 {
                     const uint32_t nv = U.f.nv[which];
@@ -3649,6 +3657,7 @@
     uint32_t prep_threads;
     bool wave_on, split_on, use_half, front_par, both;
     bool cvx_lean;
+    bool cvx_image;
     uint32_t rec_on;
     uint32_t big_quota, big_n, walk0, n_catch, n_poll;
     uint32_t n_wg, n_wg_cvx, n_wg_lean, n_wg_cvx2, n_wg_prep, n_wg_big, n_wg_half, n_wg_retry, n_wg_sweep;
@@ -3698,6 +3707,8 @@
     if (pl.front_par) pl.rec_on |= 4u;
     pl.cvx_lean = n_pairs > ctx->max_wg_small;
     if (const char* e = getenv("SURTR_CVX_LEAN")) pl.cvx_lean = n_pairs != 0 && atoi(e) != 0;
+    pl.cvx_image = true;
+    if (const char* e = getenv("SURTR_CVX_IMAGE")) pl.cvx_image = atoi(e) != 0;
     pl.prep = nullptr; pl.prep_threads = SURTR_WG;
     if (n_pairs && prep_wide) { pl.prep = k_prep_pairs_wide; pl.prep_threads = SURTR_WG_WIDE; }
     else if (n_pairs && !(pl.rec_on & 2u) && ctx->vmax < 0xFFFFu && ctx->vmin >= SURTR_PREP_MINV && (ctx->vmax + SURTR_LANES - 1u) / SURTR_LANES <= SURTR_PREP_NB)
@@ -3779,7 +3790,8 @@
     const PieceSet& M = ctx->mset; const PieceSet& C = ctx->cset;
     Pieces P{M.pos, M.loff, M.llen, M.nbr, M.vo, M.tri, M.rad, M.perm, M.posr_s, M.bsph, M.bo,
              C.pos, C.loff, C.llen, C.nbr, C.vo, C.tri, C.rad, C.perm, C.posr_s, C.bsph, C.bo, ctx->n_pieces, M.dup, C.dup,
-             M.row_s, M.iperm, M.bsph2, M.bo2, M.bsph3, M.bo3};
+             M.row_s, M.iperm, M.bsph2, M.bo2, M.bsph3, M.bo3,
+             pl.cvx_image ? C.img_vw.p : nullptr, pl.cvx_image ? C.img_re.p : nullptr, pl.cvx_image ? C.reg.p : nullptr};
     for (int i = 0; i < 16; ++i) ctx->ev_valid[i] = false;
     const uint32_t* d_pair_order = nullptr;
     if (d_pair_list && ctx->pair_order_is_list && ctx->pair_order_count == n_pairs) d_pair_order = ctx->d_pair_order;
@@ -4420,6 +4432,26 @@
         if (r.cv_n != 0) c += (r.img_fmt == IMG_NARROW || r.img_fmt == IMG_WIDE ? r.img_n : 256u) + 4u * r.mv_n + 64u;
         cost[i] = c;
     }
+    return SURTR_OK;
+}
+
+int surtr_prep_queue(surtr_ctx* ctx, uint32_t n_pairs, uint32_t* n, uint32_t* pairs)
+{
+    if (!ctx || !n) return SURTR_E_INVALID;
+    if (!ctx->have_event || !ctx->arena.cursors || n_pairs == 0 || (size_t)n_pairs > ctx->d_order.cap / 64) return SURTR_E_STATE;
+    (void)hipSetDevice(ctx->device);
+    HIPCHK(hipStreamSynchronize(ctx->stream));
+    uint32_t cnt[16];
+    HIPCHK(hipMemcpy(cnt, ctx->arena.cursors + CUR_CLS_PREP, sizeof(cnt), hipMemcpyDeviceToHost));
+    const uint32_t* porder = ctx->d_order + 16 * (ctx->d_order.cap / 64);
+    uint32_t tot = 0;
+    for (int cls = 15; cls >= 0; --cls)
+    {
+        if (cnt[cls] > n_pairs - tot) return SURTR_E_STATE;
+        if (pairs && cnt[cls]) HIPCHK(hipMemcpy(pairs + tot, porder + (size_t)cls * n_pairs, (size_t)cnt[cls] * 4, hipMemcpyDeviceToHost));
+        tot += cnt[cls];
+    }
+    *n = tot;
     return SURTR_OK;
 }
 
diff --git a/surtr_amd/engine.py b/surtr_amd/engine.py
--- a/surtr_amd/engine.py
+++ b/surtr_amd/engine.py
@@ -90,7 +90,8 @@
 
 _DERIVED = (("llen", np.uint32), ("tri", np.uint8), ("rad", np.float32), ("box", np.float32), ("perm", np.uint32),
             ("posr_s", np.float32), ("bsph", np.float32), ("bsph2", np.float32), ("bsph3", np.float32), ("iperm", np.uint32),
-            ("row_s", np.uint16), ("dup", np.uint8), ("bo", np.uint32), ("bo2", np.uint32), ("bo3", np.uint32), ("build", np.uint32))
+            ("row_s", np.uint16), ("dup", np.uint8), ("bo", np.uint32), ("bo2", np.uint32), ("bo3", np.uint32), ("build", np.uint32),
+            ("img_vw", np.uint32), ("img_re", np.uint32), ("img_reg", np.uint8))
 
 
 class Fragments(ctypes.Structure):
@@ -265,6 +266,12 @@
         self._ck(lib().surtr_event_pair_costs(self._h, ctypes.c_uint32(n_pairs), _p(out)))
         return out
 
+    def prep_queue(self, n_pairs):
+        n = ctypes.c_uint32()
+        out = np.zeros(int(n_pairs), np.uint32)
+        self._ck(lib().surtr_prep_queue(self._h, ctypes.c_uint32(int(n_pairs)), ctypes.byref(n), _p(out)))
+        return out[:n.value].copy()
+
     def queue_stats(self):
         out = (ctypes.c_uint32 * 128)()
         self._ck(lib().surtr_queue_stats(self._h, out))
@@ -608,12 +615,19 @@
             buf = np.zeros(b.value, np.uint8)
             self._ck(lib().surtr_pieces_derived(*args, _p(buf), ctypes.c_size_t(b.value), ctypes.byref(b)))
             return buf.view(dtype)
-        out = {name: get(which, dt) for which, (name, dt) in enumerate(_DERIVED)}
+        out = {name: get(which, dt) for which, (name, dt) in enumerate(_DERIVED) if set == 1 or not name.startswith("img_")}
         for name, width in (("box", 6), ("posr_s", 4), ("bsph", 4), ("bsph2", 4), ("bsph3", 4), ("row_s", 8)):
             out[name] = out[name].reshape(-1, width)
         build = out.pop("build")
         out["SB"], out["FAN"] = int(build[0]), int(build[1])
         return out
+
+    def convex_image_probe(self, solids):
+        vo, _, off, nbr = pack_solids(solids)
+        vw = np.zeros(int(vo[-1]), np.uint32); re = np.zeros(int(off[-1]), np.uint32); reg = np.zeros(len(solids), np.uint8)
+        self._ck(lib().surtr_convex_image_probe(self._h, ctypes.c_uint32(len(solids)), _p(vo), _p(off), _p(nbr), _p(vw),
+                                                _p(re if re.shape[0] else np.zeros(1, np.uint32)), _p(reg)))
+        return vw, re, reg
 
     def event_refit(self):
         self._ck(lib().surtr_event_refit(self._h))
```
